# jxx2/MetaFEM.jl

Hardware: AMD Instinct MI355X
Metric: DOF-updates/sec (assembly+CG iter) on 3D hex thermal conduction (higher is better)
Workload: dtype f64; 1 GPU; 3D thermal conduction, linear hex-8, 512x512x512 structured mesh (make_Brick): fused assembly (K + R) + 200 Jacobi-CG iterations per step; n_dof=135005697, nnz=3630961153, parallelism=single GPU

## Files before the change

include/metafem_mi355x_debug.h:

```cpp
#ifndef METAFEM_MI355X_DEBUG_H
#define METAFEM_MI355X_DEBUG_H

#include "metafem_mi355x.h"

#ifdef __cplusplus
extern "C" {
#endif

int64_t mfem_debug_sym_spmv_count(void);
long long mfem_debug_symp_fingerprint_count(void);
long long mfem_debug_symp_coded_count(void);
long long mfem_debug_symp_trim_count(void);
long long mfem_debug_symp_const_count(void);
long long mfem_debug_symp_const_steps(void);
int mfem_debug_spmv_scaled_layout(mfem_context ctx, mfem_csr A, const double* vals, const double* ssym, const double* x, double* y, double alpha, double beta,
                                  const double* dotw, double* partials_out , int32_t cap, int32_t* n_partials , int32_t* form );
int mfem_debug_set(const char* key, int64_t a, int64_t b);

int mfem_debug_lat27_cg_fused(void);
int64_t mfem_debug_lat27_pass1_bytes(mfem_csr A);
long long mfem_debug_lat27_spmv_count(void);
double mfem_debug_lat27_asymmetry(mfem_csr A);
long long mfem_debug_lat8_spmv_count(void);
double mfem_debug_lat8_asymmetry(mfem_csr A);
int mfem_debug_graph_comm_count(void);
long long mfem_debug_graph_launch_count(void);
int64_t mfem_debug_mesh_rows_count(void);
int64_t mfem_debug_mesh_direct_count(void);
int64_t mfem_debug_ws_bytes(mfem_context ctx);
int64_t mfem_debug_mesh_residual_count(void);
int64_t mfem_debug_mesh_operator_count(void);
int64_t mfem_debug_brick_operator_count(void);
int mfem_debug_brick_operator_apply_dot(mfem_context ctx, uint64_t op, const double* x, double* y, double alpha, double beta, const double* dotw,
                                        double* partials, int32_t* n_partials );
int64_t mfem_debug_mesh_ops_count(void);
int64_t mfem_debug_mesh_variants(int32_t reset);
int64_t mfem_debug_op_wave_count(int32_t kernel);
int64_t mfem_debug_sell_periodic_blocks(mfem_csr A);
int64_t mfem_debug_hex27_rows_count(void);
int64_t mfem_debug_hex27_mixed_count(void);
int64_t mfem_debug_hex27_direct_count(void);
int mfem_prof_spmv_enable(mfem_context ctx, int on);
int mfem_prof_spmv_read(mfem_context ctx, double* total_ms , int64_t* launches , int reset);
int mfem_prof_comm_enable(mfem_context ctx, int on);
int mfem_prof_comm_read(mfem_context ctx, double* halo_wait_ms , int64_t* halo_waits , double* allreduce_ms ,
                        int64_t* allreduces , int reset);
int mfem_debug_comm_selftest(mfem_context ctx, int64_t count, int32_t rounds);

unsigned long long mfem_debug_ws_address(mfem_context ctx);
long long mfem_debug_cg_ring_count(void);

int mfem_debug_ws_trial_log(mfem_context ctx, double* out4);

int mfem_debug_fail_host_alloc(int nth);


int mfem_debug_bsell_fields(mfem_csr A);
long long mfem_debug_bsell_spmv_count(void);
int mfem_debug_remainder_info(mfem_csr A, int64_t* rows , int64_t* entries , double* asym_before );
long long mfem_debug_rem_spmv_count(void);
int mfem_debug_csr_tplan(mfem_csr A, int64_t* bytes , double* build_ms );
int mfem_debug_brick_multigrid_transfer(mfem_context ctx, uint64_t mg, int32_t level, int32_t restriction, const double* in, double* out);
double* mfem_debug_brick_multigrid_coords(uint64_t mg, int32_t level, int32_t dim_id);

#ifdef __cplusplus
}
#endif
#endif
```

metafem.jl_amd/_lib.py:

```python
from __future__ import annotations

import ctypes as C
import os

import torch

_HERE = os.path.dirname(os.path.abspath(__file__))
LIB_PATH = os.path.join(_HERE, "libmetafem_mi355x.so")


class MetaFEMError(RuntimeError):
    pass


def _load():
    if not os.path.exists(LIB_PATH):
        raise ImportError(
            f"{LIB_PATH} is missing: build it with `python -c 'import __graft_entry__ as g; g.build()'` "
            "(or `make -C metafem.jl_amd/csrc`).  There is no CPU fallback.")
    return C.CDLL(LIB_PATH, mode=C.RTLD_GLOBAL)


class _Lib:

    def __init__(self, cdll):
        object.__setattr__(self, "_cdll", cdll)

    def __getattr__(self, name):
        if name.startswith("mfem_debug_set_"):
            key = name[len("mfem_debug_set_"):]
            cdll = self._cdll

            def knob(a=0, b=0, _key=key):
                if _key == "recheck_scale":
                    return cdll.mfem_debug_set(b"recheck_scale_ppm", int(round(float(a) * 1e6)), 0)
                return cdll.mfem_debug_set(_key.encode(), int(a), int(b))
            return knob
        return getattr(self._cdll, name)


lib = _Lib(_load())

c_void_p, c_int, c_int32, c_int64, c_double, c_uint64, c_uint32 = (
    C.c_void_p, C.c_int, C.c_int32, C.c_int64, C.c_double, C.c_uint64, C.c_uint32)


class SolveOptions(C.Structure):
    _fields_ = [("method", c_int32), ("precond", c_int32), ("l_or_s", c_int32), ("maxiter", c_int32),
                ("max_pass", c_int32), ("check_every", c_int32), ("converge_tol", c_double), ("seed", c_uint64),
                ("fixed_iterations", c_int32), ("scale_in_place", c_int32), ("left_precond", c_int32),
                ("cg_variant", c_int32)]


class SolveStats(C.Structure):
    _fields_ = [("passes", c_int32), ("iterations", c_int32), ("final_res", c_double), ("initial_res", c_double),
                ("solve_ms", c_double), ("converged", c_int32), ("spmv_count", c_int32)]


class ThermalParams(C.Structure):
    _fields_ = [("k", c_double), ("h", c_double), ("Tenv", c_double), ("robin_faces", c_uint32), ("fixed_faces", c_uint32),
                ("h_penalty", c_double), ("Tw", c_double)]


class ElasticityParams(C.Structure):
    _fields_ = [("lam", c_double), ("mu", c_double), ("tau", c_double), ("penalty_faces", c_uint32),
                ("traction_faces", c_uint32), ("sig", c_double * 6)]


class KvalTerm(C.Structure):
    _fields_ = [("dual_sd", c_int32), ("base_sd", c_int32), ("block", c_int32), ("reserved", c_int32)]


class ResBatchTerm(C.Structure):
    _fields_ = [("dual_sd", c_int32), ("reserved", c_int32), ("cpID_shift", c_int64)]


class VarBatchTerm(C.Structure):
    _fields_ = [("sd", c_int32), ("reserved", c_int32), ("cpID_shift", c_int64), ("x", C.c_void_p)]


class ConstTerm(C.Structure):
    _fields_ = [("dual_sd", c_int32), ("base_sd", c_int32), ("block", c_int32), ("reserved", c_int32), ("coef", c_double)]


MAX_BATCH_TERMS = 48


class MeshDirectStats(C.Structure):
    _fields_ = [(n, c_int64) for n in ("batches", "tasks", "max_batch_doubles", "max_batch_elements", "geometry_evaluations", "device_bytes",
                                       "waves_per_trip", "max_control_point_doubles", "budget_doubles", "waves_per_workgroup", "lds_bytes",
                                       "split_owners", "max_batch_owners")]


class ResSymbol(C.Structure):
    _fields_ = [("word", c_int32), ("reserved", c_int32), ("shift", c_int64), ("x", C.c_void_p)]


class AffineTerm(C.Structure):
    _fields_ = [("dual_pos", c_int32), ("dual_sd", c_int32), ("n_pairs", c_int32), ("reserved", c_int32), ("c0", c_double),
                ("sym", c_int32 * 8), ("normal", c_int32 * 8), ("coef", c_double * 8)]


MAX_RES_SYMBOLS, MAX_RES_TERMS, MAX_RES_PAIRS = 16, 48, 8


class OperatorTerm(C.Structure):
    _fields_ = [("dual_sd", c_int32), ("base_sd", c_int32), ("block", c_int32), ("reserved", c_int32), ("coef", c_double),
                ("normal_coef", c_double * 3)]


MG_MAX_LEVELS = 12


class MultigridOptions(C.Structure):
    _fields_ = [("smoother_degree", c_int32), ("coarse_degree", c_int32), ("smoothing_range", c_double), ("coarse_range", c_double),
                ("eig_steps", c_int32), ("max_levels", c_int32)]


class MultigridInfo(C.Structure):
    _fields_ = [("levels", c_int32), ("sign", c_int32), ("nx", c_int32 * 12), ("ny", c_int32 * 12), ("nz", c_int32 * 12),
                ("lambda_max", c_double * 12), ("products", c_int64 * 12), ("setup_products", c_int64), ("bytes", c_int64), ("cycles", c_int64),
                ("setups", c_int64)]


ALLREDUCE_CB = C.CFUNCTYPE(c_int, c_void_p, C.POINTER(c_double), c_int32)
EXCHANGE_CB = C.CFUNCTYPE(c_int, c_void_p, C.POINTER(c_double), C.POINTER(c_double), C.POINTER(c_double), C.POINTER(c_double), c_int64)


class CommHostOps(C.Structure):
    _fields_ = [("user", c_void_p), ("allreduce_sum", ALLREDUCE_CB), ("neighbour_exchange", EXCHANGE_CB), ("flags", c_uint32),
                ("reserved", c_uint32)]


COMM_HOST_POISON_GHOSTS = 1


class OpLayout(C.Structure):
    _fields_ = [("itg", c_int32), ("itp", c_int32), ("n_sd", c_int32), ("n_host", c_int64), ("index_base", c_int32),
                ("n_colours", c_int32), ("colour_offsets", C.POINTER(c_int64))]


P = c_void_p
SIGNATURES = {
    "mfem_abi_version": (c_int, []),
    "mfem_last_error": (C.c_char_p, []),
    "mfem_context_create": (c_int, [c_int, P, C.POINTER(P)]),
    "mfem_context_set_stream": (c_int, [P, P]),
    "mfem_context_destroy": (c_int, [P]),
    "mfem_context_sync": (c_int, [P]),
    "mfem_csr_create": (c_int, [P, c_int64, c_int64, P, c_int, P, c_int, C.POINTER(P)]),
    "mfem_csr_destroy": (c_int, [P]),
    "mfem_spmv_csr": (c_int, [P, P, P, P, P, c_double, c_double]),
    "mfem_spmv_csr_t": (c_int, [P, P, P, P, P, c_double, c_double]),
    "mfem_axpby": (c_int, [P, c_int64, c_double, P, c_double, P]),
    "mfem_dot": (c_int, [P, c_int64, P, P, C.POINTER(c_double)]),
    "mfem_nrm2": (c_int, [P, c_int64, P, C.POINTER(c_double)]),
    "mfem_rand": (c_int, [P, c_int64, c_uint64, c_uint32, P]),
    "mfem_jacobi_by_diagonal": (c_int, [P, P, P, P]),
    "mfem_jacobi2_by_column": (c_int, [P, P, P, P]),
    "mfem_jacobi_by_row": (c_int, [P, P, P, P]),
    "mfem_mat_div_jacobi": (c_int, [P, P, P, P]),
    "mfem_debug_hex27_direct_count": (c_int64, []),
    "mfem_debug_hex27_mixed_count": (c_int64, []),
    "mfem_debug_hex27_rows_count": (c_int64, []),
    "mfem_debug_mesh_rows_count": (c_int64, []),
    "mfem_debug_mesh_variants": (c_int64, [c_int32]),
    "mfem_debug_op_wave_count": (c_int64, [c_int32]),
    "mfem_debug_bsell_fields": (c_int, [P]),
    "mfem_debug_bsell_spmv_count": (c_int64, []),
    "mfem_debug_sell_periodic_blocks": (c_int64, [P]),
    "mfem_debug_symp_fingerprint_count": (C.c_longlong, []),
    "mfem_debug_symp_coded_count": (C.c_longlong, []),
    "mfem_debug_symp_trim_count": (C.c_longlong, []),
    "mfem_debug_symp_const_count": (C.c_longlong, []),
    "mfem_debug_symp_const_steps": (C.c_longlong, []),
    "mfem_debug_spmv_scaled_layout": (c_int, [P, P, P, P, P, P, c_double, c_double, P, P, c_int32, C.POINTER(c_int32), C.POINTER(c_int32)]),
    "mfem_debug_set": (c_int, [C.c_char_p, c_int64, c_int64]),
    "mfem_debug_graph_comm_count": (c_int, []),
    "mfem_debug_graph_launch_count": (C.c_longlong, []),
    "mfem_debug_cg_ring_count": (C.c_longlong, []),
    "mfem_debug_lat27_cg_fused": (c_int, []),
    "mfem_debug_lat27_pass1_bytes": (c_int64, [P]),
    "mfem_prof_spmv_enable": (c_int, [P, c_int]),
    "mfem_prof_spmv_read": (c_int, [P, C.POINTER(c_double), C.POINTER(c_int64), c_int]),
    "mfem_prof_comm_enable": (c_int, [P, c_int]),
    "mfem_prof_comm_read": (c_int, [P, C.POINTER(c_double), C.POINTER(c_int64), C.POINTER(c_double), C.POINTER(c_int64), c_int]),
    "mfem_solve": (c_int, [P, P, P, P, P, C.POINTER(SolveOptions), C.POINTER(SolveStats)]),
    "mfem_solve_set_shadow": (c_int, [P, P, c_int32]),
    "mfem_brick_create": (c_int, [P, c_int32, c_int32, c_int32, c_double, c_double, c_double, c_int32, c_int32,
                                  C.POINTER(P)]),
    "mfem_brick_destroy": (c_int, [P]),
    "mfem_brick_num_controlpoints": (c_int64, [P]),
    "mfem_brick_num_elements": (c_int64, [P]),
    "mfem_brick_coords": (P, [P, c_int32]),
    "mfem_brick_set_slab": (c_int, [P, c_int32, c_int32]),
    "mfem_brick_pattern": (c_int, [P, P, c_int32, C.POINTER(P)]),
    "mfem_pattern_build": (c_int, [P, c_int32, c_int64, c_int64, P, c_int32, c_int32, C.POINTER(P), P]),
    "mfem_csr_rowptr64": (P, [P]),
    "mfem_csr_colidx": (P, [P]),
    "mfem_csr_nnz": (c_int64, [P]),
    "mfem_csr_n": (c_int64, [P]),
    "mfem_brick_assemble_thermal": (c_int, [P, P, P, C.POINTER(ThermalParams), P]),
    "mfem_brick_residual_thermal": (c_int, [P, P, C.POINTER(ThermalParams), P, P, P]),
    "mfem_brick_assemble_elasticity": (c_int, [P, P, P, C.POINTER(ElasticityParams), P]),
    "mfem_brick_residual_elasticity": (c_int, [P, P, C.POINTER(ElasticityParams), P, P]),
    "mfem_update_basic_elements": (c_int, [P, c_int32, c_int32, c_int32, c_int64, c_int64, P, P, P, P, c_int32, P, P]),
    "mfem_update_basic_boundary": (c_int, [P, c_int32, c_int32, c_int32, c_int32, c_int64, c_int64, P, P, P, P, P, P, P,
                                          c_int32, P, P, P]),
    "mfem_op_var": (c_int, [P, C.POINTER(OpLayout), P, c_int32, c_int64, P, P, P, P, P, c_int64]),
    "mfem_op_kval": (c_int, [P, C.POINTER(OpLayout), P, c_int32, c_int32, P, P, c_int64, P, P, P, c_int64]),
    "mfem_op_res": (c_int, [P, C.POINTER(OpLayout), P, c_int32, P, c_int64, P, P, P, P, c_int64]),
    "mfem_debug_lat27_spmv_count": (c_int64, []),
    "mfem_debug_lat27_asymmetry": (C.c_double, [c_void_p]),
    "mfem_debug_lat8_spmv_count": (c_int64, []),
    "mfem_debug_lat8_asymmetry": (C.c_double, [c_void_p]),
    "mfem_spmv_solver_layout": (c_int, [P, P, P, P, P, c_double, c_double]),
    "mfem_spmv_solver_layout_dot": (c_int, [P, P, P, P, P, c_double, c_double, C.POINTER(c_double)]),
    "mfem_csr_solver_layout": (c_int, [P, P, C.POINTER(c_int32), C.POINTER(c_int32), C.POINTER(c_int64), C.POINTER(c_int64)]),
    "mfem_csr_solver_layout_entries": (c_int, [P, P, C.POINTER(c_int64), C.POINTER(c_int32)]),
    "mfem_csr_solver_layout_bytes": (c_int, [P, P, C.POINTER(c_int64)]),
    "mfem_debug_sym_spmv_count": (c_int64, []),
    "mfem_op_kval_batch": (c_int, [P, C.POINTER(OpLayout), P, c_int32, C.POINTER(KvalTerm), P, P, c_int64, c_int64, P, P, P, c_int64]),
    "mfem_op_res_batch": (c_int, [P, C.POINTER(OpLayout), P, c_int32, C.POINTER(ResBatchTerm), P, P, P, P, P, c_int64]),
    "mfem_op_var_batch": (c_int, [P, C.POINTER(OpLayout), P, c_int32, C.POINTER(VarBatchTerm), P, P, P, P, c_int64]),
    "mfem_mesh_assemble_elements": (c_int, [P, c_int32, c_int32, c_int32, c_int64, c_int64, P, P, P, P, c_int32, c_int32,
                                            C.POINTER(ConstTerm), P, c_int64, P, P, c_int64, c_int32, C.POINTER(c_int64)]),
    "mfem_mesh_assemble_elements_rows": (c_int, [P, c_int32, c_int32, c_int32, c_int64, c_int64, P, P, P, P, c_int32, c_int32,
                                                 C.POINTER(ConstTerm), c_int32, P, P, P, P, P]),
    "mfem_mesh_assemble_elements_rows_set": (c_int, [P, c_int32, c_int32, c_int32, c_int64, c_int64, P, P, P, P, c_int32, c_int32,
                                                 C.POINTER(ConstTerm), c_int32, P, P, P, P, P]),
    "mfem_mesh_direct_plan_create": (c_int, [P, c_int32, c_int64, c_int64, c_int32, P, P, P, P, c_int32, P, C.POINTER(c_uint64)]),
    "mfem_mesh_direct_plan_destroy": (c_int, [c_uint64]),
    "mfem_mesh_direct_plan_stats": (c_int, [c_uint64, C.POINTER(MeshDirectStats)]),
    "mfem_mesh_assemble_elements_direct": (c_int, [P, c_int32, c_int32, c_int32, c_int64, c_int64, P, P, P, P, c_int32, c_int32,
                                                   C.POINTER(ConstTerm), c_int32, P, c_uint64, P, c_int32]),
    "mfem_debug_mesh_direct_count": (c_int64, []),
    "mfem_debug_ws_bytes": (c_int64, [P]),
    "mfem_mesh_row_ranks": (c_int, [P, c_int32, c_int64, c_int64, c_int32, P, P, P, P, c_int32, P]),
    "mfem_mesh_assemble_facets": (c_int, [P, c_int32, c_int32, c_int32, c_int32, c_int64, c_int64, P, P, P, P, P, P, P, c_int32,
                                          c_int32, C.POINTER(ConstTerm), P, c_int64, P, P, c_int64, c_int32, C.POINTER(c_int64)]),
    "mfem_mesh_residual_elements": (c_int, [P, c_int32, c_int32, c_int32, c_int64, c_int64, P, P, P, P, c_int32, c_int32,
                                            C.POINTER(ResSymbol), c_int32, C.POINTER(AffineTerm), P, P, P]),
    "mfem_mesh_residual_facets": (c_int, [P, c_int32, c_int32, c_int32, c_int32, c_int64, c_int64, P, P, P, P, P, P, P, c_int32,
                                          c_int32, C.POINTER(ResSymbol), c_int32, C.POINTER(AffineTerm), P, P, P]),
    "mfem_debug_mesh_residual_count": (c_int64, []),
    "mfem_mesh_operator_create": (c_int, [P, c_int32, c_int32, c_int64, c_int64, c_int32, P, P, c_int32, C.POINTER(c_uint64)]),
    "mfem_mesh_operator_set_elements": (c_int, [c_uint64, c_int32, P, P, P, P, c_int32, C.POINTER(OperatorTerm)]),
    "mfem_mesh_operator_add_facets": (c_int, [c_uint64, c_int32, c_int32, c_int64, P, P, P, P, P, P, P, c_int32, C.POINTER(OperatorTerm),
                                              C.POINTER(c_int32)]),
    "mfem_mesh_operator_set_terms": (c_int, [c_uint64, c_int32, c_int32, C.POINTER(OperatorTerm)]),
    "mfem_mesh_operator_set_variable_terms": (c_int, [c_uint64, c_int32, c_int32, C.POINTER(KvalTerm), P]),
    "mfem_mesh_operator_destroy": (c_int, [c_uint64]),
    "mfem_mesh_operator_apply": (c_int, [P, c_uint64, P, P, c_double, c_double]),
    "mfem_mesh_operator_diagonal": (c_int, [P, c_uint64, P]),
    "mfem_solve_operator": (c_int, [P, c_uint64, P, P, C.POINTER(SolveOptions), C.POINTER(SolveStats)]),
    "mfem_debug_mesh_operator_count": (c_int64, []),
    "mfem_brick_operator_create": (c_int, [P, P, C.POINTER(ThermalParams), C.POINTER(c_uint64)]),
    "mfem_brick_operator_set_params": (c_int, [c_uint64, C.POINTER(ThermalParams)]),
    "mfem_brick_operator_create_elasticity": (c_int, [P, P, C.POINTER(ElasticityParams), C.POINTER(c_uint64)]),
    "mfem_brick_operator_set_elasticity_params": (c_int, [c_uint64, C.POINTER(ElasticityParams)]),
    "mfem_brick_operator_create_hex27": (c_int, [P, P, C.POINTER(ThermalParams), C.POINTER(c_uint64)]),
    "mfem_brick_operator_destroy": (c_int, [c_uint64]),
    "mfem_brick_operator_apply": (c_int, [P, c_uint64, P, P, c_double, c_double]),
    "mfem_brick_operator_diagonal": (c_int, [P, c_uint64, P]),
    "mfem_debug_brick_operator_count": (c_int64, []),
    "mfem_debug_brick_operator_apply_dot": (c_int, [P, c_uint64, P, P, c_double, c_double, P, P, C.POINTER(c_int32)]),
    "mfem_brick_multigrid_create": (c_int, [P, c_uint64, C.POINTER(MultigridOptions), C.POINTER(c_uint64)]),
    "mfem_brick_multigrid_create_elasticity": (c_int, [P, c_uint64, C.POINTER(MultigridOptions), C.POINTER(c_uint64)]),
    "mfem_brick_multigrid_setup": (c_int, [P, c_uint64]),
    "mfem_brick_multigrid_apply": (c_int, [P, c_uint64, P, P]),
    "mfem_brick_multigrid_info": (c_int, [c_uint64, C.POINTER(MultigridInfo)]),
    "mfem_brick_multigrid_destroy": (c_int, [c_uint64]),
    "mfem_debug_brick_multigrid_transfer": (c_int, [P, c_uint64, c_int32, c_int32, P, P]),
    "mfem_debug_brick_multigrid_coords": (P, [c_uint64, c_int32, c_int32]),
    "mfem_mesh_var_elements": (c_int, [P, c_int32, c_int32, c_int32, c_int64, c_int64, P, P, P, P, c_int32, c_int32,
                                       C.POINTER(VarBatchTerm), P, P, c_int64]),
    "mfem_mesh_var_facets": (c_int, [P, c_int32, c_int32, c_int32, c_int32, c_int64, c_int64, P, P, P, P, P, P, P, c_int32,
                                     c_int32, C.POINTER(VarBatchTerm), P, P, P, c_int64]),
    "mfem_mesh_res_elements": (c_int, [P, c_int32, c_int32, c_int32, c_int64, c_int64, P, P, P, P, c_int32, c_int32,
                                       C.POINTER(ResBatchTerm), P, P, P, P, P]),
    "mfem_mesh_res_facets": (c_int, [P, c_int32, c_int32, c_int32, c_int32, c_int64, c_int64, P, P, P, P, P, P, P, c_int32,
                                     c_int32, C.POINTER(ResBatchTerm), P, P, P, P, P]),
    "mfem_mesh_kval_elements": (c_int, [P, c_int32, c_int32, c_int32, c_int64, c_int64, P, P, P, P, c_int32, c_int32,
                                        C.POINTER(KvalTerm), P, P, c_int64, P, P, c_int64, c_int32, C.POINTER(c_int64)]),
    "mfem_mesh_kval_elements_rows": (c_int, [P, c_int32, c_int32, c_int32, c_int64, c_int64, P, P, P, P, c_int32, c_int32,
                                             C.POINTER(KvalTerm), P, P, c_int32, P, P, P, P, P]),
    "mfem_mesh_kval_facets": (c_int, [P, c_int32, c_int32, c_int32, c_int32, c_int64, c_int64, P, P, P, P, P, P, P, c_int32,
                                      c_int32, C.POINTER(KvalTerm), P, P, c_int64, P, P, c_int64, c_int32, C.POINTER(c_int64)]),
    "mfem_debug_mesh_ops_count": (c_int64, []),
    "mfem_comm_unique_id": (c_int, [P]),
    "mfem_comm_create": (c_int, [P, c_int32, c_int32, P, C.POINTER(P)]),
    "mfem_comm_destroy": (c_int, [P]),
    "mfem_context_set_comm": (c_int, [P, P, c_int64, c_int64, c_int32]),
    "mfem_allreduce_sum": (c_int, [P, P, c_int32]),
    "mfem_halo_exchange": (c_int, [P, P]),
    "mfem_halo_reduce": (c_int, [P, P]),
    "mfem_comm_create_host": (c_int, [P, c_int32, c_int32, C.POINTER(CommHostOps), C.POINTER(P)]),
    "mfem_csr_ncols": (c_int64, [P]),
    "mfem_csr_replan": (c_int, [P, P]),
    "mfem_csr_spmv_bytes": (c_int, [P, P, C.POINTER(c_int64), C.POINTER(c_int64)]),
    "mfem_debug_comm_selftest": (c_int, [P, c_int64, c_int32]),
    "mfem_debug_ws_address": (C.c_ulonglong, [P]),
    "mfem_debug_fail_host_alloc": (c_int, [c_int]),
    "mfem_debug_ws_trial_log": (c_int, [P, C.POINTER(C.c_double)]),
    "mfem_debug_remainder_info": (c_int, [P, C.POINTER(c_int64), C.POINTER(c_int64), C.POINTER(C.c_double)]),
    "mfem_debug_rem_spmv_count": (C.c_longlong, []),
    "mfem_debug_csr_tplan": (c_int, [P, C.POINTER(c_int64), C.POINTER(C.c_double)]),
}

for _name, (_res, _args) in SIGNATURES.items():
    _fn = getattr(lib, _name)
    _fn.restype = _res
    _fn.argtypes = _args


def check(rc: int) -> None:
    if rc != 0:
        raise MetaFEMError(f"libmetafem_mi355x rc={rc}: {lib.mfem_last_error().decode()}")
```

metafem.jl_amd/csrc/api.hip:

```cpp
#include <stdarg.h>
#include <atomic>

#include <exception>
#include <mutex>
#include <new>
#include <set>

#include "common.h"
#include <string>

static std::mutex g_ctx_mutex;
static std::set<mfem_context_s*> g_live_contexts;
bool mfem_context_alive(mfem_context_s* ctx) {
  std::lock_guard<std::mutex> lk(g_ctx_mutex);
  return g_live_contexts.count(ctx) != 0;
}

static thread_local char g_err[1024] = "";

void mfem_set_error(const char* fmt, ...) {
  va_list ap;
  va_start(ap, fmt);
  vsnprintf(g_err, sizeof(g_err), fmt, ap);
  va_end(ap);
}

int mfem_api_exception(const char* entry) noexcept {
  try {
    throw;
  } catch (const std::bad_alloc&) {
    mfem_set_error("%s: host memory exhausted (std::bad_alloc)", entry);
    return MFEM_ERR_ALLOC;
  } catch (const std::exception& e) {
    mfem_set_error("%s: internal error: %s", entry, e.what());
    return MFEM_ERR_INTERNAL;
  } catch (...) {
    mfem_set_error("%s: internal error (unknown C++ exception)", entry);
    return MFEM_ERR_INTERNAL;
  }
}

static std::atomic<int> g_fail_host_alloc{0};
extern "C" int mfem_debug_fail_host_alloc(int nth) try {
  g_fail_host_alloc.store(nth > 0 ? nth : 0);
  return MFEM_OK;
} MFEM_API_CATCH("mfem_debug_fail_host_alloc")
void mfem_host_alloc_probe() {
  int v = g_fail_host_alloc.load();
  while (v > 0) {
    if (g_fail_host_alloc.compare_exchange_weak(v, v - 1)) {
      if (v == 1) throw std::bad_alloc();
      return;
    }
  }
}

std::atomic<int> mfem_debug_epoch{0};

extern "C" int mfem_abi_version(void) { return MFEM_ABI_VERSION; }
extern "C" const char* mfem_last_error(void) { return g_err; }

int mfem_ws_release(void* raw);
static int context_allocate(mfem_context_s* c) {
  MFEM_CHECK_HIP(hipMalloc(&c->d_partials, sizeof(double) * MFEM_MAX_PARTIALS * 8));
  MFEM_CHECK_HIP(hipMalloc(&c->d_scalars, sizeof(double) * MFEM_NSCALARS));
  MFEM_CHECK_HIP(hipHostMalloc(&c->h_scalars, sizeof(double) * MFEM_NSCALARS));
  MFEM_CHECK_HIP(hipMalloc(&c->d_flags, sizeof(int32_t) * MFEM_NFLAGS));
  MFEM_CHECK_HIP(hipHostMalloc(&c->h_flags, sizeof(int32_t) * MFEM_NFLAGS));
  MFEM_CHECK_HIP(hipMemsetAsync(c->d_scalars, 0, sizeof(double) * MFEM_NSCALARS, c->stream));
  MFEM_CHECK_HIP(hipMemsetAsync(c->d_flags, 0, sizeof(int32_t) * MFEM_NFLAGS, c->stream));
  MFEM_CHECK_HIP(hipEventCreate(&c->ev0));
  MFEM_CHECK_HIP(hipEventCreate(&c->ev1));
  return MFEM_OK;
}

static void context_release(mfem_context_s* ctx) {
  if (ctx->d_partials) hipFree(ctx->d_partials);
  if (ctx->d_scalars) hipFree(ctx->d_scalars);
  if (ctx->h_scalars) hipHostFree(ctx->h_scalars);
  if (ctx->d_flags) hipFree(ctx->d_flags);
  if (ctx->h_flags) hipHostFree(ctx->h_flags);
  (void)mfem_ws_release(ctx->ws_raw);
  (void)mfem_ws_release(ctx->ws_alt_raw);
  if (ctx->prof_ev) {
    for (int i = 0; i < 2 * MFEM_PROF_PAIRS; ++i)
      if (ctx->prof_ev[i]) hipEventDestroy(ctx->prof_ev[i]);
    delete[] ctx->prof_ev;
  }
  if (ctx->ev0) hipEventDestroy(ctx->ev0);
  if (ctx->ev1) hipEventDestroy(ctx->ev1);
  for (int i = 0; i < MFEM_GRAPH_SLOTS; ++i)
    if (ctx->graph_exec[i]) hipGraphExecDestroy(ctx->graph_exec[i]);
  if (ctx->graph_ev) hipEventDestroy(ctx->graph_ev);
  if (ctx->graph_stream) hipStreamDestroy(ctx->graph_stream);
}

extern "C" int mfem_context_create(int device, void* stream, mfem_context* out) try {
  MFEM_REQUIRE(out != nullptr, "out is null");
  int ndev = 0;
  MFEM_CHECK_HIP(hipGetDeviceCount(&ndev));
  MFEM_REQUIRE(device >= 0 && device < ndev, "no such HIP device");
  MFEM_CHECK_HIP(hipSetDevice(device));
  hipDeviceProp_t prop;
  MFEM_CHECK_HIP(hipGetDeviceProperties(&prop, device));
  if (strncmp(prop.gcnArchName, "gfx950", 6) != 0) {
    mfem_set_error("libmetafem_mi355x is built for gfx950 only, device %d is %s", device, prop.gcnArchName);
    return MFEM_ERR_UNSUPPORTED;
  }
  mfem_host_alloc_probe();
  mfem_context_s* c = new mfem_context_s();
  memset(c, 0, sizeof(*c));
  c->device = device;
  c->stream = (hipStream_t)stream;
  c->num_cus = prop.multiProcessorCount;
  int rc = context_allocate(c);
  if (rc != MFEM_OK) {
    context_release(c);
    delete c;
    return rc;
  }
  {
    std::lock_guard<std::mutex> lk(g_ctx_mutex);
    g_live_contexts.insert(c);
  }
  *out = c;
  return MFEM_OK;
} MFEM_API_CATCH("mfem_context_create")

extern "C" int mfem_context_set_stream(mfem_context ctx, void* stream) try {
  MFEM_REQUIRE(ctx != nullptr, "ctx is null");
  ctx->stream = (hipStream_t)stream;
  return MFEM_OK;
} MFEM_API_CATCH("mfem_context_set_stream")

extern "C" int mfem_context_sync(mfem_context ctx) try {
  MFEM_REQUIRE(ctx != nullptr, "ctx is null");
  MFEM_CHECK_HIP(hipStreamSynchronize(ctx->stream));
  return MFEM_OK;
} MFEM_API_CATCH("mfem_context_sync")

extern "C" int mfem_context_destroy(mfem_context ctx) try {
  if (!ctx) return MFEM_OK;
  {
    std::lock_guard<std::mutex> lk(g_ctx_mutex);
    g_live_contexts.erase(ctx);
  }
  hipStreamSynchronize(ctx->stream);
  context_release(ctx);
  delete ctx;
  return MFEM_OK;
} MFEM_API_CATCH("mfem_context_destroy")

int mfem_prof_flush(mfem_context_s* ctx) {
  if (ctx->prof_used == 0) return MFEM_OK;
  MFEM_CHECK_HIP(hipEventSynchronize(ctx->prof_ev[2 * ctx->prof_used - 1]));
  for (int k = 0; k < ctx->prof_used; ++k) {
    float ms = 0.f;
    MFEM_CHECK_HIP(hipEventElapsedTime(&ms, ctx->prof_ev[2 * k], ctx->prof_ev[2 * k + 1]));
    ctx->prof_ms += ms;
  }
  ctx->prof_count += ctx->prof_used;
  ctx->prof_used = 0;
  return MFEM_OK;
}

extern "C" int mfem_prof_spmv_enable(mfem_context ctx, int on) try {
  MFEM_REQUIRE(ctx, "null ctx");
  if (on && !ctx->prof_ev) {
    ctx->prof_ev = new hipEvent_t[2 * MFEM_PROF_PAIRS]();
    for (int i = 0; i < 2 * MFEM_PROF_PAIRS; ++i) MFEM_CHECK_HIP(hipEventCreate(&ctx->prof_ev[i]));
  }
  if (!on) {
    int rc = mfem_prof_flush(ctx);
    if (rc) return rc;
  }
  ctx->prof_on = on ? 1 : 0;
  return MFEM_OK;
} MFEM_API_CATCH("mfem_prof_spmv_enable")

extern "C" int mfem_prof_spmv_read(mfem_context ctx, double* total_ms, int64_t* launches, int reset) try {
  MFEM_REQUIRE(ctx && total_ms && launches, "null argument");
  int rc = mfem_prof_flush(ctx);
  if (rc) return rc;
  *total_ms = ctx->prof_ms;
  *launches = ctx->prof_count;
  if (reset) {
    ctx->prof_ms = 0.0;
    ctx->prof_count = 0;
  }
  return MFEM_OK;
} MFEM_API_CATCH("mfem_prof_spmv_read")

uint64_t mfem_next_csr_serial() {
  static std::atomic<uint64_t> next{1};
  return next.fetch_add(1);
}

void mfem_graphs_invalidate(mfem_context_s* ctx) {
  for (int i = 0; i < MFEM_GRAPH_SLOTS; ++i)
    if (ctx->graph_exec[i]) {
      hipGraphExecDestroy(ctx->graph_exec[i]);
      ctx->graph_exec[i] = nullptr;
      ctx->graph_key[i] = 0;
    }
}

static std::atomic<size_t> g_ws_align{0}, g_ws_offset{0};
extern "C" int mfem_debug_set_ws_placement(long long align, long long offset) try {
  g_ws_align = align > 0 ? (size_t)align : 0;
  g_ws_offset = offset > 0 ? (size_t)offset : 0;
  return MFEM_OK;
} MFEM_API_CATCH("mfem_debug_set_ws_placement")
static int ws_alloc(mfem_context_s* ctx, void** raw, size_t bytes) {
  (void)ctx;
  *raw = nullptr;
  MFEM_CHECK_HIP(hipMalloc(raw, bytes));
  return MFEM_OK;
}
static int ws_free(void* raw) {
  if (raw) MFEM_CHECK_HIP(hipFree(raw));
  return MFEM_OK;
}
int mfem_ws_release(void* raw) { return ws_free(raw); }
extern "C" int64_t mfem_debug_ws_bytes(mfem_context ctx) { return ctx ? (int64_t)ctx->ws_bytes : 0; }
extern "C" unsigned long long mfem_debug_ws_address(mfem_context ctx) { return ctx ? (unsigned long long)(uintptr_t)ctx->ws : 0ull; }
#include <chrono>
static double now_ms() { return std::chrono::duration<double, std::milli>(std::chrono::steady_clock::now().time_since_epoch()).count(); }
int mfem_ws_next_candidate(mfem_context_s* ctx) {
  const bool verbose = getenv("MFEM_WS_TRIAL_VERBOSE") != nullptr;
  double t0 = now_ms();
  MFEM_CHECK_HIP(hipStreamSynchronize(ctx->stream));
  if (verbose) fprintf(stderr, "ws trial: sync %.1f ms\n", now_ms() - t0);
  const size_t need = ctx->ws_bytes + g_ws_align + g_ws_offset;
  if (ctx->ws_alt_raw) {
    t0 = now_ms();
    {
      int rcf = ws_free(ctx->ws_raw);
      if (rcf) return rcf;
    }
    if (verbose) fprintf(stderr, "ws trial: free %.1f ms\n", now_ms() - t0);
    ctx->ws = ctx->ws_raw = nullptr;
  }
  size_t freeb = 0, totalb = 0;
  void* raw = nullptr;
  bool ok = hipMemGetInfo(&freeb, &totalb) == hipSuccess && freeb >= need + ((size_t)4 << 30);
  t0 = now_ms();
  if (ok && ws_alloc(ctx, &raw, need) != MFEM_OK) ok = false;
  if (verbose) fprintf(stderr, "ws trial: alloc %.1f ms\n", now_ms() - t0);
  if (!ok) {
    (void)hipGetLastError();
    if (!ctx->ws_raw) {
      ctx->ws = ctx->ws_alt;
      ctx->ws_raw = ctx->ws_alt_raw;
      ctx->ws_alt = ctx->ws_alt_raw = nullptr;
    }
    return MFEM_OK;
  }
  if (ctx->ws_raw) {
    ctx->ws_alt = ctx->ws;
    ctx->ws_alt_raw = ctx->ws_raw;
  }
  ctx->ws_raw = raw;
  uintptr_t p = (uintptr_t)raw;
  if (g_ws_align) p = (p + g_ws_align - 1) / g_ws_align * g_ws_align;
  ctx->ws = (void*)(p + g_ws_offset);
  ctx->ws_try += 1;
  return MFEM_OK;
}
int mfem_ws_decide(mfem_context_s* ctx, bool keep_current) {
  MFEM_CHECK_HIP(hipStreamSynchronize(ctx->stream));
  if (ctx->ws_alt_raw) {
    if (keep_current) {
      int rcf = ws_free(ctx->ws_alt_raw);
      if (rcf) return rcf;
    } else {
      int rcf = ws_free(ctx->ws_raw);
      if (rcf) return rcf;
      ctx->ws = ctx->ws_alt;
      ctx->ws_raw = ctx->ws_alt_raw;
    }
  }
  ctx->ws_alt = ctx->ws_alt_raw = nullptr;
  ctx->ws_try = 99;
  return MFEM_OK;
}
int mfem_ws_reserve(mfem_context_s* ctx, size_t bytes) {
  if (bytes <= ctx->ws_bytes) return MFEM_OK;
  MFEM_CHECK_HIP(hipStreamSynchronize(ctx->stream));
  int rcf = ws_free(ctx->ws_raw);
  if (!rcf) rcf = ws_free(ctx->ws_alt_raw);
  ctx->ws = ctx->ws_raw = ctx->ws_alt = ctx->ws_alt_raw = nullptr;
  ctx->ws_try = 0;
  ctx->ws_bytes = 0;
  if (rcf) return rcf;
  rcf = ws_alloc(ctx, &ctx->ws_raw, bytes + g_ws_align + g_ws_offset);
  if (rcf) return rcf;
  uintptr_t p = (uintptr_t)ctx->ws_raw;
  if (g_ws_align) p = (p + g_ws_align - 1) / g_ws_align * g_ws_align;
  ctx->ws = (void*)(p + g_ws_offset);
  ctx->ws_bytes = bytes;
  return MFEM_OK;
}

extern "C" {
int mfem_debug_set_spmv(int, int);
int mfem_debug_set_ell(int);
int mfem_debug_set_sell(int);
int mfem_debug_set_lat27(int);
int mfem_debug_set_lat8(int);
int mfem_debug_set_layout_min_rows(int64_t, int64_t);
int mfem_debug_set_graphs(int, int64_t);
int mfem_debug_set_idrs(int);
int mfem_debug_set_bicgstabl(int);
int mfem_debug_set_gmres(int);
int mfem_debug_set_vec_grid(int);
int mfem_debug_set_halo_overlap(int);
int mfem_debug_set_hex27(int);
int mfem_debug_set_elasticity(int);
int mfem_debug_set_hex8_thermal(int);
int mfem_debug_set_ws_placement(long long, long long);
int mfem_debug_set_ws_trial(int);
int mfem_debug_set_cg_streaming(int);
int mfem_debug_set_cg_ring(int);
int mfem_debug_set_cg_single_max_rows(int64_t);
int mfem_debug_set_csr_strips(int, int64_t);
int mfem_debug_set_remainder(int);
int mfem_debug_set_recheck_scale(double);
int mfem_debug_set_bsell(int);
}
extern int g_mesh_gather_rows, g_mesh_abl, g_mesh_stage_min_itp, g_mesh_term_matrix;
extern int g_op_wave_forms, g_op_wave_min_itp;
extern int64_t g_mesh_direct_budget;
extern "C" int mfem_debug_set(const char* key, int64_t a, int64_t b) try {
  MFEM_REQUIRE(key, "null key");
  const std::string k(key);
  if (k == "spmv") return mfem_debug_set_spmv((int)a, (int)b);
  if (k == "ell") return mfem_debug_set_ell((int)a);
  if (k == "sell") return mfem_debug_set_sell((int)a);
  if (k == "lat27") return mfem_debug_set_lat27((int)a);
  if (k == "lat8") return mfem_debug_set_lat8((int)a);
  if (k == "layout_min_rows") return mfem_debug_set_layout_min_rows(a, b);
  if (k == "graphs") return mfem_debug_set_graphs((int)a, b);
  if (k == "idrs") return mfem_debug_set_idrs((int)a);
  if (k == "bicgstabl") return mfem_debug_set_bicgstabl((int)a);
  if (k == "gmres") return mfem_debug_set_gmres((int)a);
  if (k == "vec_grid") return mfem_debug_set_vec_grid((int)a);
  if (k == "halo_overlap") return mfem_debug_set_halo_overlap((int)a);
  if (k == "hex27") return mfem_debug_set_hex27((int)a);
  if (k == "elasticity") return mfem_debug_set_elasticity((int)a);
  if (k == "hex8_thermal") return mfem_debug_set_hex8_thermal((int)a);
  if (k == "ws_placement") return mfem_debug_set_ws_placement((long long)a, (long long)b);
  if (k == "ws_trial") return mfem_debug_set_ws_trial((int)a);
  if (k == "cg_streaming") return mfem_debug_set_cg_streaming((int)a);
  if (k == "cg_ring") return mfem_debug_set_cg_ring((int)a);
  if (k == "cg_single_max_rows") return mfem_debug_set_cg_single_max_rows(a);
  if (k == "csr_strips") return mfem_debug_set_csr_strips((int)a, b);
  if (k == "remainder") return mfem_debug_set_remainder((int)a);
  if (k == "mesh_gather_rows") { g_mesh_gather_rows = (int)a; return MFEM_OK; }
  if (k == "bsell") return mfem_debug_set_bsell((int)a);
  if (k == "op_wave_forms") { g_op_wave_forms = (int)a; g_op_wave_min_itp = b > 0 ? (int)b : 10; return MFEM_OK; }
  if (k == "mesh_stage_min_itp") { g_mesh_stage_min_itp = a > 0 ? (int)a : 16; return MFEM_OK; }
  if (k == "mesh_term_matrix") { g_mesh_term_matrix = (int)a; return MFEM_OK; }
  if (k == "mesh_direct_budget") { g_mesh_direct_budget = a > 0 ? a : 0; return MFEM_OK; }
  if (k == "mesh_abl") { g_mesh_abl = (int)a; return MFEM_OK; }
  if (k == "recheck_scale_ppm") return mfem_debug_set_recheck_scale((double)a * 1e-6);
  mfem_set_error("mfem_debug_set: unknown key '%s'", key);
  return MFEM_ERR_INVALID;
} MFEM_API_CATCH("mfem_debug_set")
```

metafem.jl_amd/csrc/common.h:

```cpp
#pragma once
#include <hip/hip_runtime.h>
#include <atomic>
#include <mutex>
#include <unordered_map>
#include <stdint.h>
#include <stdio.h>
#include <string.h>

#if defined(__HIP_DEVICE_COMPILE__) && !defined(__gfx950__)
#error "metafem_mi355x is written for gfx950 (MI355X) only: counted s_waitcnt vmcnt(k) pipelines assume loads and stores share one in-order counter, global_load_lds_dwordx4 and v_mfma_f64 are used directly -- build with --offload-arch=gfx950"
#endif
#include "../../include/metafem_mi355x.h"
#include "../../include/metafem_mi355x_debug.h"
#include "csr_decide.h"
#include "sell_decide.h"
#include "lat_decide.h"

#define MFEM_WAVE 64
#define MFEM_BLOCK 256
#define MFEM_MAX_PARTIALS 4096
static_assert(LAT_MAX_GATHER_GRID == MFEM_MAX_PARTIALS, "a workgroup of the tiles' gather pass writes one partial sum");
#define MFEM_NFLAGS 80
#define MFEM_NSCALARS 4096

void mfem_set_error(const char* fmt, ...);

int mfem_api_exception(const char* entry) noexcept;
#define MFEM_API_CATCH(entry) catch (...) { return mfem_api_exception(entry); }
void mfem_host_alloc_probe();

#define MFEM_CHECK_HIP(expr)                                                                  \
  do {                                                                                        \
    hipError_t _e = (expr);                                                                   \
    if (_e != hipSuccess) {                                                                   \
      mfem_set_error("%s:%d: %s -> %s", __FILE__, __LINE__, #expr, hipGetErrorString(_e));    \
      return MFEM_ERR_HIP;                                                                    \
    }                                                                                         \
  } while (0)

#define MFEM_REQUIRE(cond, msg)                                      \
  do {                                                               \
    if (!(cond)) {                                                   \
      mfem_set_error("%s:%d: %s (%s)", __FILE__, __LINE__, msg, #cond); \
      return MFEM_ERR_INVALID;                                       \
    }                                                                \
  } while (0)

#define MFEM_CHECK_LAUNCH() MFEM_CHECK_HIP(hipGetLastError())

template <typename T> struct __attribute__((visibility("hidden"))) DevBuf {
  T* p = nullptr;
  DevBuf() = default;
  DevBuf(DevBuf&& o) noexcept : p(o.release()) {}
  DevBuf& operator=(DevBuf&& o) noexcept { if (this != &o) { reset(); p = o.release(); } return *this; }
  DevBuf(const DevBuf&) = delete;
  DevBuf& operator=(const DevBuf&) = delete;
  ~DevBuf() { reset(); }
  hipError_t alloc(size_t count) { reset(); return hipMalloc((void**)&p, sizeof(T) * count); }
  void reset() { if (p) (void)hipFree(p); p = nullptr; }
  T* release() { T* q = p; p = nullptr; return q; }
  operator T*() const { return p; }
};

struct mfem_comm_s;

#define MFEM_MAX_ZONES 8
struct SpmvPart {
  int part;
  int nz;
  int64_t lo[MFEM_MAX_ZONES], hi[MFEM_MAX_ZONES];
};
__host__ __device__ __forceinline__ bool spmv_part_skip(const SpmvPart& P, int64_t r0, int64_t r1) {
  if (P.part == 0) return false;
  bool bnd = false;
  for (int z = 0; z < P.nz; ++z) bnd = bnd || (r0 < P.hi[z] && r1 > P.lo[z]);
  return P.part == 1 ? bnd : !bnd;
}


#define MFEM_GRAPH_SLOTS 4
struct mfem_context_s {
  int device;
  hipStream_t stream;
  int num_cus;
  double* d_partials;
  double* d_scalars;
  double* h_scalars;
  int32_t* d_flags;
  int32_t* h_flags;
  void* ws;
  void* ws_raw;
  size_t ws_bytes;
  int ws_try;
  void* ws_alt;
  void* ws_alt_raw;
  float ws_try_ms;
  float ws_log[4];
  const double* shadow;
  int32_t shadow_count;
  mfem_comm_s* comm;
  int64_t halo_plane_len;
  int32_t halo_fields;
  hipEvent_t ev0, ev1;
  int prof_on;
  int prof_used;
  hipEvent_t* prof_ev;
  double prof_ms;
  int64_t prof_count;
  hipGraphExec_t graph_exec[MFEM_GRAPH_SLOTS];
  uint64_t graph_key[MFEM_GRAPH_SLOTS];
  int graph_next;
  hipStream_t graph_stream;
  hipEvent_t graph_ev;
  int graph_active;
  int force_csr;
  int probe_active;
};
#define MFEM_PROF_PAIRS 1024
int mfem_prof_flush(mfem_context_s* ctx);

struct mfem_operator_head;
struct mfem_csr_s {
  mfem_context_s* ctx;
  uint64_t serial;
  int64_t n, nnz;
  const void* rowptr;
  int rowptr_bits;
  const int32_t* colidx;
  int index_base;
  int32_t max_row_nnz;
  CsrPlan plan;
  int nb_F, nb_checked;
  int64_t rb_ntiles;
  int64_t rb_elided;
  int32_t* rb_rows;
  uint8_t* cw_elide;
  int32_t lat_m1, lat_m2, lat_fields;
  int32_t lat_m0, lat_plo, lat_gw;
  int32_t lat_inferred;
  uint16_t* diag_off;
  void* owned_rowptr;
  void* owned_colidx;
  int64_t x_offset;
  int64_t ncols;
  int ell_state, ell_K;
  int64_t ell_npad;
  int32_t* ell_cols;
  const double* ell_src;
  double* ell_vals;
  int dia_state, dia_classes;
  void* dia_dev;
  int32_t* dia_flags;
  int32_t dia_regular_blocks;
  int dia_triples;
  int sym_state;
  int64_t sym_c0, sym_c1;
  int sym_cls;
  int sym_S;
  int64_t sym_mx, sym_myz;
  int ell_bound_mode;
  int dia_kernel;
  int symp_state;
  int symp_m1, symp_m2;
  int64_t symp_PL;
  int symp_p0, symp_p1;
  int symp_NS, symp_NPk;
  int symp_B;
  int symp_trim;
  int symp_DC;
  int symp_dneg;
  int symp_CS;
  int symp_cs_last;
  int64_t symp_flagged, symp_flagged_last;
  double symp_cst[27];
  int symp_ccode;
  int symp_dc_last;
  double* symp_vals;
  SellLayout sell;
  LatTiles lat27, lat8;
  int lat_refused;
  int rem_active;
  int64_t rem_nrows, rem_nent, rem_cap_rows, rem_cap_ent;
  int32_t* rem_rows;
  int64_t* rem_ptr;
  int32_t* rem_len;
  int32_t* rem_col;
  double* rem_val;
  unsigned long long* rem_cnt;
  void* rem_sort_tmp;
  size_t rem_sort_bytes;
  double rem_asym_before;
  int64_t rem_last_rows, rem_last_ent;
  struct mfem_tplan_s* tplan;
  struct mfem_operator_head* op;
  double* op_scratch;
  const double* op_dsc;
  uint64_t op_epoch;
};
struct mfem_tplan_s {
  mfem_csr_s* AT;
  void* perm;
  int perm_bits;
  double* vals;
  int64_t bytes;
  double build_ms;
};
static inline CsrShape mfem_csr_shape(const mfem_csr_s* A) { return {A->n, A->nnz, A->max_row_nnz}; }
template <typename F> static inline auto mfem_by_rowptr(const mfem_csr_s* A, F&& f) { return A->rowptr_bits == 64 ? f(int64_t{}) : f(int32_t{}); }
int mfem_tplan_get(mfem_context_s* ctx, mfem_csr_s* A, mfem_tplan_s** out);
void mfem_tplan_free(mfem_csr_s* A);
int mfem_tplan_gather(mfem_context_s* ctx, const mfem_tplan_s* P, const double* src, double* valsT, const double* d1, const double* d2);
bool mfem_rem_enabled();
bool mfem_rem_diag();
void mfem_rem_clear(mfem_csr_s* A);
void mfem_rem_free(mfem_csr_s* A);
int mfem_rem_build(mfem_context_s* ctx, mfem_csr_s* A, const double* vals, int n_fields, const double* y1, const double* y2, const double* scale,
                   double gate, bool* built);
int mfem_rem_apply(mfem_context_s* ctx, mfem_csr_s* A, const double* x, const double* dsc, double* y, double alpha, const double* dotw,
                   double* partials, int* n_partials, const int32_t* done_flag);
int64_t mfem_rem_design_bytes(const mfem_csr_s* A);
int mfem_spmv_lat8_launch(mfem_context_s* ctx, mfem_csr_s* A, const double* vals, const double* x, double* y, double alpha, double beta,
                          const double* dotw, double* partials, int* n_partials, const int32_t* done_flag, int part);
int64_t mfem_lat8_design_bytes(const mfem_csr_s* A);
int64_t mfem_lat8_entries(const mfem_csr_s* A);
int mfem_lattice_hint_from_row0(mfem_context_s* ctx, mfem_csr_s* A);
static inline LatShape mfem_lat_shape(const mfem_csr_s* A, int64_t min_rows) {
  return {A->n, A->ncols, A->max_row_nnz, A->lat_m0, A->lat_m1, A->lat_m2, A->lat_fields, A->lat_plo, A->lat_gw, min_rows};
}
static inline void mfem_lat_unbind(mfem_csr_s* A, LatTiles& T) {
  if (T.vals) A->rem_active = 0;
  T.vals = T.dump = nullptr;
  T.src = T.dsc = nullptr;
}
int mfem_sym_probe(mfem_context_s* ctx, mfem_csr_s* A, LatTiles* T, const double* vals, double* scratch, double amax, double* asym, int rem_fields);
int mfem_spmv_lat27_launch(mfem_context_s* ctx, mfem_csr_s* A, const double* vals, const double* x, double* y, double alpha,
                           double beta, const double* dotw, double* partials, int* n_partials, const int32_t* done_flag, int part);
int64_t mfem_lat27_design_bytes(const mfem_csr_s* A);
int64_t mfem_lat27_entries(const mfem_csr_s* A);
int mfem_node_block_fields(mfem_context_s* ctx, mfem_csr_s* A);
int mfem_spmv_sell_launch(mfem_context_s* ctx, mfem_csr_s* A, const double* vals, const double* x, double* y, double alpha,
                          double beta, const double* dotw, double* partials, int* n_partials, const int32_t* done_flag, int part);
int mfem_ell_diag(mfem_context_s* ctx, mfem_csr_s* A, double* d);
int mfem_spmv_ell_launch(mfem_context_s* ctx, mfem_csr_s* A, const double* vals, const double* x, double* y, double alpha,
                         double beta, const double* dotw, double* partials, int* n_partials, const int32_t* done_flag,
                         const SpmvPart& part);
struct SpmvArgs {
  const double* x; double* y; double alpha, beta; const double* dotw; double* partials; int* n_partials; const int32_t* done_flag; const SpmvPart& part;
};
__attribute__((visibility("hidden"))) int mfem_spmv_csr_launch(mfem_context_s* ctx, mfem_csr_s* A, const double* vals, const double* x, double* y, double alpha,
                                                             double beta, const double* dotw, double* partials, int* n_partials, const int32_t* done_flag,
                                                             const SpmvPart& part);
__attribute__((visibility("hidden"))) CsrKnobs mfem_csr_knobs();

enum mfem_layout : int32_t { MFEM_LAYOUT_CSR = 0, MFEM_LAYOUT_ELL = 1, MFEM_LAYOUT_DIA = 2, MFEM_LAYOUT_SELL = 3, MFEM_LAYOUT_LAT27 = 4, MFEM_LAYOUT_LAT8 = 5,
                             MFEM_LAYOUT_OPERATOR = 6  };
struct mfem_layout_plan_s {
  mfem_layout tile, rows;
  size_t tile_bytes, rows_bytes;
};
int mfem_layout_plan(mfem_context_s* ctx, mfem_csr_s* A, bool is_cg, bool allow_tiles, mfem_layout_plan_s* P);
int mfem_layout_bind(mfem_context_s* ctx, mfem_csr_s* A, mfem_layout mode, const double* vals, double* buf, const double* dsc, const double* ssym,
                     double* scratch, bool allow_rem);
mfem_layout mfem_layout_bound(const mfem_csr_s* A, const double* vals);
void mfem_layout_unbind(mfem_csr_s* A);
void mfem_layout_drop(mfem_csr_s* A);

int mfem_ws_reserve(mfem_context_s* ctx, size_t bytes);
int mfem_ws_next_candidate(mfem_context_s* ctx);
int mfem_ws_decide(mfem_context_s* ctx, bool keep_current);
uint64_t mfem_next_csr_serial();
bool mfem_context_alive(mfem_context_s* ctx);
void mfem_graphs_invalidate(mfem_context_s* ctx);
extern std::atomic<int> mfem_debug_epoch;

__device__ __forceinline__ double wave_reduce_sum(double v) {
#pragma unroll
  for (int off = 32; off > 0; off >>= 1) v += __shfl_down(v, off, MFEM_WAVE);
  return v;
}

__device__ __forceinline__ void mfem_lds_barrier() { asm volatile("s_waitcnt lgkmcnt(0)\n\ts_barrier" ::: "memory"); }

__device__ __forceinline__ bool mfem_xcd_tile(int tcount, int& tsub) {
  const int chunk = (tcount + 7) >> 3;
  tsub = (int)(blockIdx.x & 7) * chunk + (int)(blockIdx.x >> 3);
  return !((int)(blockIdx.x >> 3) >= chunk || tsub >= tcount);
}

__device__ __forceinline__ double block_reduce_sum(double v, double* smem ) {
  v = wave_reduce_sum(v);
  const int lane = threadIdx.x & 63, w = threadIdx.x >> 6;
  __syncthreads();
  if (lane == 0) smem[w] = v;
  __syncthreads();
  double r = 0.0;
  if (threadIdx.x == 0) {
    const int nw = (blockDim.x + 63) >> 6;
    for (int i = 0; i < nw; ++i) r += smem[i];
  }
  __syncthreads();
  return r;
}

static inline int mfem_resident_per_cu(const void* kernel, int block_threads, size_t dyn_lds, int fallback) {
  static std::mutex mu;
  static std::unordered_map<const void*, int> cache;
  std::lock_guard<std::mutex> lk(mu);
  auto it = cache.find(kernel);
  if (it != cache.end()) return it->second;
  int occ = 0;
  const hipError_t e = hipOccupancyMaxActiveBlocksPerMultiprocessor(&occ, kernel, block_threads, dyn_lds);
  const int v = (e == hipSuccess && occ >= 1) ? occ : fallback;
  cache[kernel] = v;
  return v;
}
static inline int mfem_grid_for(int64_t work_items, int per_block, int cap) {
  int64_t g = (work_items + per_block - 1) / per_block;
  if (g < 1) g = 1;
  if (g > cap) g = cap;
  return (int)g;
}
```

metafem.jl_amd/csrc/spmv_ell.h:

```cpp
#pragma once
#include <vector>

#include "layouts.h"
#include "spmv_symp.h"
#include "symp_trim_decide.h"
#include "symp_const_decide.h"

#define ELL_B 128
__host__ __device__ __forceinline__ int64_t ell_base(int64_t r, int K) { return (r >> 7) * ((int64_t)K * ELL_B) + (r & (ELL_B - 1)); }

typedef double e_d2 __attribute__((ext_vector_type(2)));
typedef int e_i2 __attribute__((ext_vector_type(2)));
typedef double u_d2 __attribute__((ext_vector_type(2), aligned(8)));

#define DIA_MAXD 96
#define DIA_MAXC 4
struct DiaOffsets {
  int ncls;
  int D[DIA_MAXC];
  int32_t off[DIA_MAXC][DIA_MAXD];
};

struct SympGeom {
  int64_t PL, nx;
  int m1, m2, p0, p1, NS, NPk;
  int nseg;
  int B, NR;
  int DC;
  long long unit;
  int ms1, ms2;
  int rim_pp;
  int64_t rim_rows, rim_units;
};
struct SympConst {
  double v[27];
  int32_t code, valid;
};
#define SPC_COUNT_AT 20
#define SPC_REF_AT 22
static_assert(SPC_REF_AT % 2 == 0 && SPC_REF_AT * 4 + sizeof(SympConst) <= MFEM_NFLAGS * 4, "the reference row must fit the context's flags");
struct SympTail {
  int on, K;
  int rim;
  int64_t n, npad, lo, hi;
  const DiaOffsets* Op;
  const int32_t* flags;
  const int32_t* cols;
  const double* ell;
};

#if defined(DV_ABL) && DV_ABL == 1
#define DIA_ST(p, v) do { if ((v) == 1.2345e300) __builtin_nontemporal_store((v), (p)); } while (0)
#elif defined(DV_ABL) && DV_ABL == 3
#define DIA_ST(p, v) (*(p) = (v))
#else
#define DIA_ST(p, v) __builtin_nontemporal_store((v), (p))
#endif
#define SYM_LD(p) __builtin_nontemporal_load(p)

template <int RPT, int U, bool TRIPLES>
__device__ __forceinline__ void dia_rows(int64_t r, int64_t n, int64_t npad, int K, const DiaOffsets& O,
                                         const int32_t* __restrict__ flags, const int32_t* __restrict__ cols,
                                         const double* __restrict__ vals, const double* __restrict__ x, double* __restrict__ y,
                                         double alpha, double beta, const double* __restrict__ dotw, int xcd, double& dot_acc,
                                         int64_t skip_lo = 0, int64_t skip_hi = 0) {
  constexpr int H = RPT / 2;
  const double* v = vals + ell_base(r, K);
  e_d2 acc[H];
  double xself0 = 0.0, xself1 = 0.0;
  bool have_self = false;
#pragma unroll
  for (int h = 0; h < H; ++h) acc[h] = (e_d2){0.0, 0.0};
  const int64_t blk = r / (64 * RPT) * (RPT / 2);
  const int cls = __builtin_amdgcn_readfirstlane(flags[blk]) - 1;
  bool interior = cls >= 0;
  if (RPT == 4) interior = interior && ((blk + 1) * 128 < npad) && flags[blk + 1] == cls + 1;
  const int32_t* off = O.off[cls < 0 ? 0 : cls];
  const int D = O.D[cls < 0 ? 0 : cls];
  if (interior && TRIPLES && RPT == 2) {
    for (int s = 0; s < D; s += 3) {
      const e_d2 va = __builtin_nontemporal_load(reinterpret_cast<const e_d2*>(v + s * ELL_B));
      const e_d2 vb = __builtin_nontemporal_load(reinterpret_cast<const e_d2*>(v + (s + 1) * ELL_B));
      const e_d2 vc = __builtin_nontemporal_load(reinterpret_cast<const e_d2*>(v + (s + 2) * ELL_B));
      const u_d2* xp = reinterpret_cast<const u_d2*>(x + r + off[s]);
      const u_d2 xa = xp[0], xb = xp[1];
      acc[0].x += va.x != 0.0 ? va.x * xa.x : 0.0;
      acc[0].y += va.y != 0.0 ? va.y * xa.y : 0.0;
      acc[0].x += vb.x != 0.0 ? vb.x * xa.y : 0.0;
      acc[0].y += vb.y != 0.0 ? vb.y * xb.x : 0.0;
      acc[0].x += vc.x != 0.0 ? vc.x * xb.x : 0.0;
      acc[0].y += vc.y != 0.0 ? vc.y * xb.y : 0.0;
      if (off[s + 1] == 0) {
        xself0 = xa.y;
        xself1 = xb.x;
        have_self = true;
      }
    }
  } else if (interior) {
    int s = 0;
    for (; s + U <= D; s += U) {
      e_d2 vv[U][H];
      u_d2 xx[U][H];
#pragma unroll
      for (int u = 0; u < U; ++u)
#pragma unroll
        for (int h = 0; h < H; ++h) {
          vv[u][h] = __builtin_nontemporal_load(reinterpret_cast<const e_d2*>(v + (s + u) * ELL_B) + h);
          xx[u][h] = *(reinterpret_cast<const u_d2*>(x + r + off[s + u]) + h);
        }
#pragma unroll
      for (int u = 0; u < U; ++u)
#pragma unroll
        for (int h = 0; h < H; ++h) {
          acc[h].x += vv[u][h].x != 0.0 ? vv[u][h].x * xx[u][h].x : 0.0;
          acc[h].y += vv[u][h].y != 0.0 ? vv[u][h].y * xx[u][h].y : 0.0;
        }
    }
    for (; s < D; ++s)
#pragma unroll
      for (int h = 0; h < H; ++h) {
        const e_d2 vv = __builtin_nontemporal_load(reinterpret_cast<const e_d2*>(v + s * ELL_B) + h);
        const u_d2 xx = *(reinterpret_cast<const u_d2*>(x + r + off[s]) + h);
        acc[h].x += vv.x != 0.0 ? vv.x * xx.x : 0.0;
        acc[h].y += vv.y != 0.0 ? vv.y * xx.y : 0.0;
      }
  } else {
    const int32_t* c = cols + ell_base(r, K);
    for (int s = 0; s < K; ++s)
#pragma unroll
      for (int h = 0; h < H; ++h) {
        if (r + 2 * h >= npad) continue;
        const e_d2 vv = __builtin_nontemporal_load(reinterpret_cast<const e_d2*>(v + s * ELL_B) + h);
        const e_i2 cc = __builtin_nontemporal_load(reinterpret_cast<const e_i2*>(c + s * ELL_B) + h);
        acc[h].x += vv.x * x[cc.x];
        acc[h].y += vv.y * x[cc.y];
      }
  }
#pragma unroll
  for (int h = 0; h < H; ++h) {
    const int64_t rr = r + 2 * h;
    if (rr >= n) break;
    double y0 = alpha * acc[h].x, y1 = alpha * acc[h].y;
    const bool one = rr < skip_lo || rr >= skip_hi;
    const bool two = rr + 1 < n && (rr + 1 < skip_lo || rr + 1 >= skip_hi);
    if (beta != 0.0) {
      if (one) y0 += beta * y[rr];
      if (two) y1 += beta * y[rr + 1];
    }
    if (one) y[rr] = y0;
    if (two) y[rr + 1] = y1;
    if (dotw) {
      if (RPT == 2 && have_self && dotw == x) {
        if (one) dot_acc += y0 * xself0;
        if (two) dot_acc += y1 * xself1;
      } else {
        if (one) dot_acc += y0 * dotw[rr];
        if (two) dot_acc += y1 * dotw[rr + 1];
      }
    }
  }
}

struct EllKnobs {
  std::atomic<int> enable{1};
  std::atomic<int> dia{1};
  std::atomic<int> symp_trim{0};
  std::atomic<int> symp_const{0};
  std::atomic<int> grid_mult{6};
  std::atomic<int> shared_x{1};
  std::atomic<int> xcd{0};
  std::atomic<int> symp_coded{1};
  std::atomic<int> sym{1};
  std::atomic<int> symp{1};
  std::atomic<int> symp_bands{0};
  std::atomic<int> symp_tail{1};
  std::atomic<int> symp_direct{1};
  std::atomic<int> dia_pipe{1};
  std::atomic<int> dia_fast{1};
  std::atomic<int> symp_fingerprint{1};
};
extern EllKnobs g_ell;
extern std::atomic<int64_t> g_layout_min_rows_dia, g_layout_min_rows_cols;

enum DiaKernel : int { DIA_NONE = 0, DIA_ROWS, DIA_ROWS_TRIPLES, DIA_SYM27, DIA_SYMP };
DiaKernel mfem_dia_kernel_wanted(const mfem_csr_s* A, DiaKernel refused = DIA_NONE, bool* direct = nullptr);
int mfem_dia_plan(mfem_context_s* ctx, mfem_csr_s* A);
int mfem_dia_copy(mfem_context_s* ctx, mfem_csr_s* A, const double* vals, double* buf, const double* dsc, const double* ssym, const SympGeom& G,
                  double* pvals, double* rim, bool want_fp, bool* fp_made, unsigned char* sflags = nullptr, bool* flags_made = nullptr);
int mfem_dia_launch(mfem_context_s* ctx, mfem_csr_s* A, bool triples, int cap, const SpmvArgs& a);
int mfem_dia_launch_outside(mfem_context_s* ctx, mfem_csr_s* A, const SpmvArgs& a, double* partials, int64_t lo, int64_t hi, int* ngrid);
void mfem_sym_plan(mfem_csr_s* A, const int32_t* off, int lc, int64_t m2, int64_t PL, int64_t run_lo, int64_t run_hi);
bool mfem_sym_wanted(const mfem_csr_s* A, DiaKernel k);
SympGeom mfem_symp_geom(const mfem_context_s* ctx, const mfem_csr_s* A);
int64_t mfem_symp_steps(const mfem_csr_s* A, int B = 0, int trim = -1);
int mfem_symp_bands_wanted(const mfem_csr_s* A);
int mfem_symp_bands(const mfem_csr_s* A);
int mfem_symp_trim_wanted(const mfem_csr_s* A);
int mfem_symp_trim(const mfem_csr_s* A);
int64_t mfem_symp_copy_doubles(const mfem_csr_s* A, int B, int trim);
int64_t mfem_symp_swept_rows(const mfem_csr_s* A);
int mfem_symp_coded_wanted(DiaKernel k, bool fast, const double* ssym);
int mfem_symp_coded(const mfem_csr_s* A);
bool mfem_dia_fill_fast(const mfem_csr_s* A, const double* dsc, bool direct);
int64_t mfem_sym_entries(const mfem_context_s* ctx, const mfem_csr_s* A, DiaKernel k);
int mfem_sym_verdict(mfem_context_s* ctx, mfem_csr_s* A, DiaKernel k, const double* buf, double* pvals, const SympGeom& G, bool direct, bool fp_made, bool* ok,
                     bool* dc_refused, int* dneg, bool flags_made = false, SympConst* cst = nullptr, int64_t* flagged = nullptr);
unsigned char* mfem_symp_flags_of(double* pvals, const SympGeom& G);
int mfem_sym_launch(mfem_context_s* ctx, mfem_csr_s* A, DiaKernel k, const SpmvArgs& a);
```

metafem.jl_amd/csrc/spmv_ell.hip:

```cpp
#include "blas1.h"
#include "spmv_ell.h"

std::atomic<int64_t> g_layout_min_rows_dia{262144};
std::atomic<int64_t> g_layout_min_rows_cols{1000000};
#define LAT27_MIN_ROWS 180000
std::atomic<int64_t> g_layout_min_rows_lat27{LAT27_MIN_ROWS};
extern "C" int mfem_debug_set_layout_min_rows(int64_t diagonal_slots, int64_t explicit_columns) try {
  ++mfem_debug_epoch;
  g_layout_min_rows_dia = diagonal_slots;
  g_layout_min_rows_cols = explicit_columns;
  g_layout_min_rows_lat27 = explicit_columns < LAT27_MIN_ROWS ? explicit_columns : LAT27_MIN_ROWS;
  return MFEM_OK;
} MFEM_API_CATCH("mfem_debug_set_layout_min_rows")

EllKnobs g_ell;
extern "C" int mfem_debug_set_ell(int enable) try {
  ++mfem_debug_epoch;
  g_ell.enable = enable & 1;
  g_ell.dia = (enable & 2) ? 0 : 1;
  g_ell.symp_trim = (enable & 4) ? 2 : (enable & 8) ? 1 : 0;
  g_ell.symp_const = (enable & 16) ? 2 : (enable & 32) ? 1 : 0;
  if ((enable >> 8) & 255) g_ell.grid_mult = (enable >> 8) & 255;
  g_ell.shared_x = ((enable >> 16) & 15) == 8 ? 0 : 1;
  g_ell.xcd = (enable >> 20) & 1;
  g_ell.symp_coded = ((enable >> 21) & 1) ? 0 : 1;
  g_ell.sym = ((enable >> 22) & 1) ? 0 : 1;
  g_ell.symp = ((enable >> 23) & 1) ? 0 : 1;
  g_ell.symp_bands = ((enable >> 24) & 1) ? 1 : ((enable >> 25) & 1) ? 2 : 0;
  g_ell.symp_tail = ((enable >> 26) & 1) ? 0 : 1;
  g_ell.symp_direct = ((enable >> 27) & 1) ? 0 : 1;
  g_ell.dia_pipe = ((enable >> 28) & 1) ? 0 : 1;
  g_ell.dia_fast = ((enable >> 29) & 1) ? 0 : 1;
  g_ell.symp_fingerprint = ((enable >> 30) & 1) ? 0 : 1;
  return MFEM_OK;
} MFEM_API_CATCH("mfem_debug_set_ell")

template <typename RP>
__global__ __launch_bounds__(MFEM_BLOCK) void k_ell_cols(int64_t n, int64_t npad, int K, const RP* __restrict__ rowptr,
                                                           const int32_t* __restrict__ col, int base, int32_t* __restrict__ out) {
  const int64_t stride = (int64_t)gridDim.x * blockDim.x;
  for (int64_t r = blockIdx.x * (int64_t)blockDim.x + threadIdx.x; r < npad; r += stride) {
    int64_t lo = 0;
    int len = 0;
    if (r < n) {
      lo = (int64_t)rowptr[r] - base;
      len = (int)((int64_t)rowptr[r + 1] - base - lo);
    }
    const int32_t self = (int32_t)(r < n ? r : 0);
    for (int s = 0; s < K; ++s) out[ell_base(r, K) + s * ELL_B] = s < len ? col[lo + s] - base : self;
  }
}

template <typename RP>
__global__ __launch_bounds__(MFEM_BLOCK) void k_ell_vals_lds(int64_t n, int64_t npad, int K, const RP* __restrict__ rowptr,
                                                               const double* __restrict__ vals, int base, double* __restrict__ out,
                                                               const int32_t* __restrict__ col, const double* __restrict__ dsc) {
  extern __shared__ double lds[];
  const int lane = threadIdx.x & 63, w = threadIdx.x >> 6, nw = blockDim.x >> 6;
  double* T = lds + (size_t)w * 64 * K;
  const int64_t ntiles = npad >> 6;
  for (int64_t tile = (int64_t)blockIdx.x * nw + w; tile < ntiles; tile += (int64_t)gridDim.x * nw) {
    const int64_t r0 = tile << 6, r = r0 + lane;
    const int64_t rend = (r0 + 64 < n) ? r0 + 64 : n;
    int64_t lo = 0;
    int len = 0;
    if (r < n) {
      lo = (int64_t)rowptr[r] - base;
      len = (int)((int64_t)rowptr[r + 1] - base - lo);
    }
    const int64_t s0 = r0 < n ? (int64_t)rowptr[r0] - base : 0;
    const int cnt = r0 < n ? (int)((int64_t)rowptr[rend] - base - s0) : 0;
    constexpr int NB = 28;
    for (int i0 = lane; i0 < cnt; i0 += 64 * NB) {
      double tv[NB];
#pragma unroll
      for (int u = 0; u < NB; ++u) {
        const int i = i0 + 64 * u;
        tv[u] = i < cnt ? vals[s0 + i] : 0.0;
        if (dsc && i < cnt) tv[u] /= dsc[col[s0 + i] - base];
      }
#pragma unroll
      for (int u = 0; u < NB; ++u) {
        const int i = i0 + 64 * u;
        if (i < cnt) T[i] = tv[u];
      }
    }
    __builtin_amdgcn_wave_barrier();
    __builtin_amdgcn_s_waitcnt(0xC07F);
    const int off = (int)(lo - s0);
    for (int s = 0; s < K; ++s) out[ell_base(r, K) + s * ELL_B] = s < len ? T[off + s] : 0.0;
    __builtin_amdgcn_wave_barrier();
  }
}

template <int RPT, int U>
__global__ __launch_bounds__(MFEM_BLOCK) void k_spmv_ell(int64_t n, int64_t npad, int K, const int32_t* __restrict__ cols,
                                                           const double* __restrict__ vals, const double* __restrict__ x,
                                                           double* __restrict__ y, double alpha, double beta,
                                                           const double* __restrict__ dotw, double* __restrict__ partials,
                                                           const int32_t* __restrict__ done_flag, SpmvPart part) {
  __shared__ double red[4];
  if (done_flag && done_flag[0]) return;
  double dot_acc = 0.0;
  const int64_t stride = (int64_t)gridDim.x * blockDim.x * RPT;
  for (int64_t r = (blockIdx.x * (int64_t)blockDim.x + threadIdx.x) * RPT; r < n; r += stride) {
    if (spmv_part_skip(part, r, r + RPT)) continue;
    const double* v = vals + ell_base(r, K);
    const int32_t* c = cols + ell_base(r, K);
    if (RPT == 1) {
      double acc = 0.0;
      int s = 0;
      for (; s + U <= K; s += U) {
        double vv[U];
        int32_t cc[U];
#pragma unroll
        for (int u = 0; u < U; ++u) {
          vv[u] = __builtin_nontemporal_load(v + (s + u) * ELL_B);
          cc[u] = __builtin_nontemporal_load(c + (s + u) * ELL_B);
        }
#pragma unroll
        for (int u = 0; u < U; ++u) acc += vv[u] * x[cc[u]];
      }
      for (; s < K; ++s) acc += __builtin_nontemporal_load(v + s * ELL_B) * x[__builtin_nontemporal_load(c + s * ELL_B)];
      double yv = alpha * acc;
      if (beta != 0.0) yv += beta * y[r];
      y[r] = yv;
      if (dotw) dot_acc += yv * dotw[r];
    } else {
      e_d2 acc = {0.0, 0.0};
      int s = 0;
      for (; s + U <= K; s += U) {
        e_d2 vv[U];
        e_i2 cc[U];
#pragma unroll
        for (int u = 0; u < U; ++u) {
          vv[u] = __builtin_nontemporal_load(reinterpret_cast<const e_d2*>(v + (s + u) * ELL_B));
          cc[u] = __builtin_nontemporal_load(reinterpret_cast<const e_i2*>(c + (s + u) * ELL_B));
        }
#pragma unroll
        for (int u = 0; u < U; ++u) {
          acc.x += vv[u].x * x[cc[u].x];
          acc.y += vv[u].y * x[cc[u].y];
        }
      }
      for (; s < K; ++s) {
        const e_d2 v1 = __builtin_nontemporal_load(reinterpret_cast<const e_d2*>(v + s * ELL_B));
        const e_i2 c1 = __builtin_nontemporal_load(reinterpret_cast<const e_i2*>(c + s * ELL_B));
        acc.x += v1.x * x[c1.x];
        acc.y += v1.y * x[c1.y];
      }
      double y0 = alpha * acc.x, y1 = alpha * acc.y;
      const bool two = r + 1 < n;
      if (beta != 0.0) {
        y0 += beta * y[r];
        if (two) y1 += beta * y[r + 1];
      }
      y[r] = y0;
      if (two) y[r + 1] = y1;
      if (dotw) {
        dot_acc += y0 * dotw[r];
        if (two) dot_acc += y1 * dotw[r + 1];
      }
    }
  }
  if (partials) {
    const double b = block_reduce_sum(dot_acc, red);
    if (threadIdx.x == 0) partials[blockIdx.x] = b;
  }
}

__global__ __launch_bounds__(MFEM_BLOCK) void k_ell_diag(int64_t n, int K, const DiaOffsets* __restrict__ Op,
                                                           const int32_t* __restrict__ flags, const int32_t* __restrict__ cols,
                                                           const double* __restrict__ vals, double* __restrict__ d) {
  const int64_t stride = (int64_t)gridDim.x * blockDim.x;
  for (int64_t r = blockIdx.x * (int64_t)blockDim.x + threadIdx.x; r < n; r += stride) {
    const int64_t b = ell_base(r, K);
    const int cls = flags ? flags[r >> 7] - 1 : -1;
    double out = 1.0;
    if (cls >= 0) {
      const int D = Op->D[cls];
      for (int s = 0; s < D; ++s)
        if (Op->off[cls][s] == 0) {
          const double v = vals[b + s * ELL_B];
          if (v != 0.0) out = fabs(v);
          break;
        }
    } else {
      for (int s = 0; s < K; ++s)
        if (cols[b + s * ELL_B] == (int32_t)r) {
          const double v = vals[b + s * ELL_B];
          if (v != 0.0) out = fabs(v);
          break;
        }
    }
    d[r] = out;
  }
}

static int ell_plan_columns(mfem_context_s* ctx, mfem_csr_s* A) {
  A->ell_state = -1;
  const int K = A->max_row_nnz;
  if (A->n < 1 || K < 1 || K > 128) return MFEM_OK;
  const int64_t npad = (A->n + ELL_B - 1) & ~(int64_t)(ELL_B - 1);
  if ((double)K * (double)npad > 1.10 * (double)A->nnz + 64.0 * K) return MFEM_OK;
  MFEM_CHECK_HIP(hipMalloc(&A->ell_cols, sizeof(int32_t) * (size_t)K * (size_t)npad));
  const int grid = mfem_grid_for(npad, MFEM_BLOCK, ctx->num_cus * 16);
  mfem_by_rowptr(A, [&](auto t) {
    hipLaunchKernelGGL(k_ell_cols<decltype(t)>, dim3(grid), dim3(MFEM_BLOCK), 0, ctx->stream, A->n, npad, K, (const decltype(t)*)A->rowptr, A->colidx,
                       A->index_base, A->ell_cols);
  });
  MFEM_CHECK_LAUNCH();
  A->ell_K = K;
  A->ell_npad = npad;
  A->ell_state = 1;
  return MFEM_OK;
}
int mfem_ell_plan(mfem_context_s* ctx, mfem_csr_s* A) {
  if (A->ell_state != 0) return MFEM_OK;
  if (A->n < g_layout_min_rows_dia && A->n < g_layout_min_rows_cols) return MFEM_OK;
  struct Undo {
    mfem_csr_s* A;
    ~Undo() {
      if (!A) return;
      mfem_ell_free(A);
      A->sym_state = A->symp_state = 0;
    }
  } undo{A};
  int rc = ell_plan_columns(ctx, A);
  if (!rc && A->ell_state == 1) rc = mfem_dia_plan(ctx, A);
  if (!rc) undo.A = nullptr;
  return rc;
}

bool mfem_dia_layout_planned(const mfem_csr_s* A) { return A->ell_state == 1 && g_ell.enable && A->dia_state == 1 && g_ell.dia; }
DiaKernel mfem_dia_kernel_wanted(const mfem_csr_s* A, DiaKernel refused, bool* direct) {
  DiaKernel k = DIA_ROWS;
  if (A->dia_triples && g_ell.shared_x) {
    k = DIA_ROWS_TRIPLES;
    if (refused != DIA_SYM27 && mfem_sym_wanted(A, DIA_SYM27)) k = DIA_SYM27;
    if (refused == DIA_NONE && mfem_sym_wanted(A, DIA_SYMP)) k = DIA_SYMP;
  }
  if (direct) *direct = k == DIA_SYMP && g_ell.symp_direct;
  return k;
}
#define SYMP_BANDS2_MIN_ROWS 100000000
int mfem_symp_bands_wanted(const mfem_csr_s* A) {
  if (g_ell.symp_bands) return g_ell.symp_bands;
  return A->symp_state == 1 && (int64_t)(A->symp_p1 - A->symp_p0) * A->symp_PL >= SYMP_BANDS2_MIN_ROWS ? 2 : 1;
}
int mfem_symp_bands(const mfem_csr_s* A) { return A->symp_B ? A->symp_B : mfem_symp_bands_wanted(A); }
#define SYMP_TRIM_MIN_ROWS 16000000
int mfem_symp_trim_wanted(const mfem_csr_s* A) {
  if (g_ell.symp_trim) return g_ell.symp_trim == 1 ? 1 : 0;
  return A->symp_state == 1 && (int64_t)(A->symp_p1 - A->symp_p0) * A->symp_PL >= SYMP_TRIM_MIN_ROWS ? 1 : 0;
}
int mfem_symp_trim(const mfem_csr_s* A) { return A->symp_B ? A->symp_trim : mfem_symp_trim_wanted(A); }
static std::atomic<long long> g_symp_trim_binds{0};
extern "C" long long mfem_debug_symp_trim_count(void) { return g_symp_trim_binds; }
int mfem_symp_coded_wanted(DiaKernel k, bool fast, const double* ssym) { return k == DIA_SYMP && fast && ssym && g_ell.symp_coded ? 1 : 0; }
int mfem_symp_coded(const mfem_csr_s* A) { return A->symp_vals ? A->symp_DC : A->symp_dc_last; }
static std::atomic<long long> g_symp_coded_binds{0};
extern "C" long long mfem_debug_symp_coded_count(void) { return g_symp_coded_binds; }
static std::atomic<long long> g_symp_const_binds{0}, g_symp_const_steps{0};
extern "C" long long mfem_debug_symp_const_count(void) { return g_symp_const_binds; }
extern "C" long long mfem_debug_symp_const_steps(void) { return g_symp_const_steps; }
size_t mfem_ell_vals_bytes(const mfem_csr_s* A) {
  if (A->ell_state != 1 || !g_ell.enable) return 0;
  const bool dia = mfem_dia_layout_planned(A);
  if (A->n < (dia ? g_layout_min_rows_dia : g_layout_min_rows_cols)) return 0;
  size_t bytes = sizeof(double) * (size_t)A->ell_K * (size_t)A->ell_npad;
  if (dia && mfem_dia_kernel_wanted(A) == DIA_SYMP) {
    size_t pm = 0;
    for (int B = 1; B <= SP_BMAX; ++B)
      for (int trim = 0; trim <= 1; ++trim) pm = std::max(pm, sizeof(double) * (size_t)mfem_symp_copy_doubles(A, B, trim));
    bytes += pm;
  }
  return bytes;
}
static int dia_bind(mfem_context_s* ctx, mfem_csr_s* A, const double* vals, double* buf, const double* dsc, const double* ssym) {
  bool direct = false, fp_made = false, flags_made = false;
  SympConst cst{};
  int64_t flagged = 0;
  DiaKernel k = mfem_dia_kernel_wanted(A, DIA_NONE, &direct);
  A->symp_trim = mfem_symp_trim_wanted(A);
  A->symp_B = mfem_symp_bands_wanted(A);
  A->symp_DC = mfem_symp_coded_wanted(k, mfem_dia_fill_fast(A, dsc, direct), ssym);
  A->symp_dneg = 0;
  double* pvals = buf + (size_t)A->ell_K * (size_t)A->ell_npad;
  SympGeom G = k == DIA_SYMP ? mfem_symp_geom(ctx, A) : SympGeom{};
  auto rim_of = [&](const SympGeom& g) -> double* { return k == DIA_SYMP && g.rim_units > 0 ? pvals + (int64_t)g.NR * g.NPk * (g.p1 - g.p0) * sp_step(g.B, g.DC) : nullptr; };
  auto flags_of = [&](const SympGeom& g) -> unsigned char* { return k == DIA_SYMP && direct && g_ell.symp_const != 2 ? mfem_symp_flags_of(pvals, g) : nullptr; };
  int rc = mfem_dia_copy(ctx, A, vals, buf, dsc, ssym, G, direct ? pvals : nullptr, rim_of(G), g_ell.symp_fingerprint != 0, &fp_made, flags_of(G), &flags_made);
  while (!rc && (k == DIA_SYMP || k == DIA_SYM27)) {
    bool ok = false, dc_refused = false;
    rc = mfem_sym_verdict(ctx, A, k, buf, pvals, G, direct, fp_made, &ok, &dc_refused, &A->symp_dneg, flags_made, &cst, &flagged);
    if (rc) break;
    if (dc_refused) {
      A->symp_DC = 0;
      G = mfem_symp_geom(ctx, A);
      rc = mfem_dia_copy(ctx, A, vals, buf, dsc, ssym, G, pvals, rim_of(G), g_ell.symp_fingerprint != 0, &fp_made, flags_of(G), &flags_made);
      continue;
    }
    if (ok) break;
    if (k == DIA_SYMP && direct) rc = mfem_dia_copy(ctx, A, vals, buf, dsc, ssym, SympGeom{}, nullptr, nullptr, false, &fp_made);
    k = mfem_dia_kernel_wanted(A, k);
  }
  if (rc) return rc;
  A->ell_vals = buf;
  A->ell_src = vals;
  A->ell_bound_mode = 2;
  A->dia_kernel = k;
  A->symp_vals = k == DIA_SYMP ? pvals : nullptr;
  if (k != DIA_SYMP) A->symp_B = A->symp_DC = A->symp_trim = 0;
  if (!A->symp_DC) A->symp_dneg = 0;
  A->symp_CS = 0;
  A->symp_flagged = 0;
  if (k == DIA_SYMP) {
    const int64_t steps = mfem_symp_steps(A);
    if (!flags_made) flagged = 0;
    bool mirror = fp_made || flagged == 0;
    for (int sl = 0; sl < 13 && mirror && flagged > 0; ++sl) mirror = memcmp(&cst.v[sl], &cst.v[26 - sl], sizeof(double)) == 0;
    A->symp_CS = spc_form(flags_made && mirror, flags_made && cst.valid != 0, flagged, steps, g_ell.symp_const == 2, g_ell.symp_const == 1);
    A->symp_flagged = flagged;
    memcpy(A->symp_cst, cst.v, sizeof(A->symp_cst));
    A->symp_ccode = cst.code;
    A->symp_cs_last = A->symp_CS;
    A->symp_flagged_last = flagged;
    g_symp_const_steps = flagged;
    if (A->symp_CS) ++g_symp_const_binds;
    A->symp_dc_last = A->symp_DC;
    if (A->symp_DC) ++g_symp_coded_binds;
    if (G.rim_units > 0) ++g_symp_trim_binds;
  }
  return MFEM_OK;
}

int mfem_ell_bind(mfem_context_s* ctx, mfem_csr_s* A, const double* vals, double* buf, const double* dsc, const double* ssym) {
  mfem_ell_unbind(A);
  if (A->ell_state != 1 || !g_ell.enable || !buf) return MFEM_OK;
  if (mfem_dia_layout_planned(A)) return dia_bind(ctx, A, vals, buf, dsc, ssym);
  int waves = 4;
  while (waves > 1 && sizeof(double) * 64 * (size_t)A->ell_K * waves > 64 * 1024) waves >>= 1;
  const size_t lds = sizeof(double) * 64 * (size_t)A->ell_K * waves;
  const int64_t ntiles = A->ell_npad >> 6;
  int grid = (int)((ntiles + waves - 1) / waves);
  if (grid > ctx->num_cus * 16) grid = ctx->num_cus * 16;
  mfem_by_rowptr(A, [&](auto t) {
    hipLaunchKernelGGL(k_ell_vals_lds<decltype(t)>, dim3(grid), dim3(64 * waves), lds, ctx->stream, A->n, A->ell_npad, A->ell_K,
                       (const decltype(t)*)A->rowptr, vals, A->index_base, buf, A->colidx, dsc);
  });
  MFEM_CHECK_LAUNCH();
  A->ell_vals = buf;
  A->ell_src = vals;
  A->ell_bound_mode = 1;
  return MFEM_OK;
}
void mfem_ell_unbind(mfem_csr_s* A) {
  A->ell_bound_mode = A->dia_kernel = DIA_NONE;
  A->ell_vals = A->symp_vals = nullptr;
  A->ell_src = nullptr;
  A->symp_B = A->symp_DC = A->symp_dneg = A->symp_trim = A->symp_CS = 0;
  A->symp_flagged = 0;
}
void mfem_ell_free(mfem_csr_s* A) {
  if (A->ell_cols) hipFree(A->ell_cols);
  if (A->dia_flags) hipFree(A->dia_flags);
  if (A->dia_dev) hipFree(A->dia_dev);
  A->ell_cols = nullptr;
  A->dia_flags = nullptr;
  A->dia_dev = nullptr;
  A->ell_state = A->dia_state = 0;
}
int mfem_ell_diag(mfem_context_s* ctx, mfem_csr_s* A, double* d) {
  if (!A->ell_vals) return MFEM_ERR_INVALID;
  const int grid = mfem_grid_for(A->n, MFEM_BLOCK, ctx->num_cus * 16);
  hipLaunchKernelGGL(k_ell_diag, dim3(grid), dim3(MFEM_BLOCK), 0, ctx->stream, A->n, A->ell_K, (const DiaOffsets*)A->dia_dev,
                     A->ell_bound_mode == 2 ? A->dia_flags : nullptr, A->ell_cols, A->ell_vals, d);
  MFEM_CHECK_LAUNCH();
  return MFEM_OK;
}

static std::atomic<int64_t> g_sym_launches{0};
extern "C" int64_t mfem_debug_sym_spmv_count(void) { return g_sym_launches; }
int mfem_spmv_ell_launch(mfem_context_s* ctx, mfem_csr_s* A, const double* vals, const double* x, double* y, double alpha, double beta,
                         const double* dotw, double* partials, int* n_partials, const int32_t* done_flag, const SpmvPart& part) {
  if (!A->ell_vals || vals != A->ell_src) return 0;
  int cap = ctx->num_cus * g_ell.grid_mult;
  if (cap > MFEM_MAX_PARTIALS) cap = MFEM_MAX_PARTIALS;
  if (part.part != 0) cap /= 2;
  if (part.part == 2) {
    int64_t rows = 0;
    for (int z = 0; z < part.nz; ++z) rows += part.hi[z] - part.lo[z];
    const int64_t want = rows / 512 + 2 * part.nz + 1;
    if (want < cap) cap = (int)want;
  }
  const SpmvArgs a{x, y, alpha, beta, dotw, partials, n_partials, done_flag, part};
  int rc = MFEM_OK;
  switch (A->ell_bound_mode == 2 ? A->dia_kernel : DIA_NONE) {
    case DIA_SYMP:
    case DIA_SYM27:
      if (part.part != 2) ++g_sym_launches;
      rc = mfem_sym_launch(ctx, A, (DiaKernel)A->dia_kernel, a);
      break;
    case DIA_ROWS_TRIPLES:
    case DIA_ROWS: rc = mfem_dia_launch(ctx, A, A->dia_kernel == DIA_ROWS_TRIPLES, cap, a); break;
    default: {
      const int grid = mfem_grid_for((A->n + 1) / 2, MFEM_BLOCK, cap);
      hipLaunchKernelGGL((k_spmv_ell<2, 1>), dim3(grid), dim3(MFEM_BLOCK), 0, ctx->stream, A->n, A->ell_npad, A->ell_K, A->ell_cols, A->ell_vals, x,
                         y, alpha, beta, dotw, partials, done_flag, part);
      MFEM_CHECK_LAUNCH();
      if (n_partials && partials) *n_partials = grid;
    }
  }
  return rc ? rc : 1;
}

int64_t mfem_ell_entries(const mfem_context_s* ctx, const mfem_csr_s* A, int32_t* sweep) {
  const DiaKernel k = mfem_dia_layout_planned(A) ? mfem_dia_kernel_wanted(A) : DIA_NONE;
  if (sweep) *sweep = k == DIA_SYMP ? 2 : k == DIA_SYM27 ? 1 : 0;
  return k == DIA_SYMP || k == DIA_SYM27 ? mfem_sym_entries(ctx, A, k) : (int64_t)A->ell_K * A->ell_npad;
}
int64_t mfem_ell_design_bytes(const mfem_context_s* ctx, const mfem_csr_s* A) {
  int32_t sym = 0;
  const int64_t ent = mfem_ell_entries(ctx, A, &sym);
  if (!mfem_dia_layout_planned(A)) return ent * 12 + A->n * 16;
  const int64_t reg = (int64_t)A->dia_regular_blocks * 128;
  int64_t b = ent * 8 + A->n * 16 + (A->n > reg ? A->n - reg : 0) * (int64_t)A->ell_K * 4;
  if (sym == 2) b += mfem_symp_steps(A) * (int64_t)sp_xn(mfem_symp_bands(A)) * 8 - mfem_symp_swept_rows(A) * 8;
  return b;
}
```

metafem.jl_amd/csrc/spmv_sym.hip:

```cpp
#include "blas1.h"
#include "spmv_ell.h"

#define SYM_ROWS 512
#define SYM_THREADS (SYM_ROWS / 2)
#define SYM_WG_PER_CU 3
__global__ __launch_bounds__(SYM_THREADS) void k_spmv_sym27(int64_t n, int64_t npad, int K, const DiaOffsets* __restrict__ Op,
                                                             const int32_t* __restrict__ flags, const int32_t* __restrict__ cols,
                                                             const double* __restrict__ vals, const double* __restrict__ x,
                                                             double* __restrict__ y, double alpha, double beta,
                                                             const double* __restrict__ dotw, double* __restrict__ partials,
                                                             const int32_t* __restrict__ done_flag, int64_t c0, int64_t c1, int S, int nsteps, int cls, int gs,
                                                             int part) {
  __shared__ __attribute__((aligned(16))) double hist[9][SYM_ROWS];
  __shared__ __attribute__((aligned(16))) double exch[4][SYM_ROWS];
  __shared__ double red[16];
  if (done_flag && done_flag[0]) return;
  const int32_t* off = Op->off[cls];
  const int tid = threadIdx.x;
  double dot_acc = 0.0;
  const int tile = blockIdx.x % S, seg = blockIdx.x / S;
  const int nseg = gs / S + (tile < gs % S ? 1 : 0);
  const int seg_len = part == 2 ? 0 : (nsteps + nseg - 1) / nseg;
  bool have_hist = false;
  e_d2 up_next[4] = {{0.0, 0.0}, {0.0, 0.0}, {0.0, 0.0}, {0.0, 0.0}};
  {
    const int64_t chunk = c0 + tile + (int64_t)S * ((int64_t)seg * seg_len);
    if (part != 2 && seg * seg_len < nsteps && chunk < c1) {
      const double* v = vals + ell_base(chunk * SYM_ROWS + 2 * tid, K);
#pragma unroll
      for (int u = 0; u < 4; ++u) up_next[u] = SYM_LD(reinterpret_cast<const e_d2*>(v + (14 + u) * ELL_B));
    }
  }
  for (int it = 0; it < seg_len; ++it) {
    const int step = seg * seg_len + it;
    const int64_t chunk = c0 + tile + (int64_t)S * step;
    if (step >= nsteps || chunk >= c1) break;
    const int64_t r = chunk * SYM_ROWS + 2 * tid;
    const double* v = vals + ell_base(r, K);
    e_d2 acc = {0.0, 0.0};
    e_d2 up[4];
#pragma unroll
    for (int u = 0; u < 4; ++u) {
      up[u] = up_next[u];
      *reinterpret_cast<e_d2*>(&exch[u][2 * tid]) = up[u];
    }
    __syncthreads();
    auto slot = [&](int s, const double* tab, int lp, bool ok) -> e_d2 {
      e_d2 w;
      if (ok && lp >= 0 && lp + 1 < SYM_ROWS) {
        w.x = tab[lp];
        w.y = tab[lp + 1];
      } else {
        w = SYM_LD(reinterpret_cast<const e_d2*>(v + s * ELL_B));
      }
      return w;
    };
#define SYM_RUN(va, vb, vc, s0)                                          \
  {                                                                      \
    const u_d2* xp = reinterpret_cast<const u_d2*>(x + r + off[s0]);     \
    const u_d2 xa = xp[0], xb = xp[1];                                   \
    acc.x += va.x != 0.0 ? va.x * xa.x : 0.0;                            \
    acc.y += va.y != 0.0 ? va.y * xa.y : 0.0;                            \
    acc.x += vb.x != 0.0 ? vb.x * xa.y : 0.0;                            \
    acc.y += vb.y != 0.0 ? vb.y * xb.x : 0.0;                            \
    acc.x += vc.x != 0.0 ? vc.x * xb.x : 0.0;                            \
    acc.y += vc.y != 0.0 ? vc.y * xb.y : 0.0;                            \
    if (s0 == 12) {                                                      \
      xself0 = xa.y;                                                     \
      xself1 = xb.x;                                                     \
    }                                                                    \
  }
    double xself0 = 0.0, xself1 = 0.0;
    const int lph = 2 * tid + S * SYM_ROWS;
#pragma unroll
    for (int s = 0; s < 9; s += 3) {
      const e_d2 va = slot(s, hist[8 - s], lph + off[s], have_hist);
      const e_d2 vb = slot(s + 1, hist[7 - s], lph + off[s + 1], have_hist);
      const e_d2 vc = slot(s + 2, hist[6 - s], lph + off[s + 2], have_hist);
      SYM_RUN(va, vb, vc, s);
    }
    {
      const e_d2 va = slot(9, exch[3], 2 * tid + off[9], true);
      const e_d2 vb = slot(10, exch[2], 2 * tid + off[10], true);
      const e_d2 vc = slot(11, exch[1], 2 * tid + off[11], true);
      SYM_RUN(va, vb, vc, 9);
    }
    {
      e_d2 va;
      va.y = up[0].x;
      if (tid > 0) va.x = exch[0][2 * tid - 1];
      else va.x = v[12 * ELL_B];
      const e_d2 vb = SYM_LD(reinterpret_cast<const e_d2*>(v + 13 * ELL_B));
      SYM_RUN(va, vb, up[0], 12);
    }
    SYM_RUN(up[1], up[2], up[3], 15);
    if (it + 1 < seg_len && step + 1 < nsteps && chunk + S < c1) {
      const double* vn = vals + ell_base((chunk + S) * SYM_ROWS + 2 * tid, K);
#pragma unroll
      for (int u = 0; u < 4; ++u) up_next[u] = SYM_LD(reinterpret_cast<const e_d2*>(vn + (14 + u) * ELL_B));
    }
    __syncthreads();
#pragma unroll
    for (int s = 18; s < 27; s += 3) {
      const e_d2 va = SYM_LD(reinterpret_cast<const e_d2*>(v + s * ELL_B));
      const e_d2 vb = SYM_LD(reinterpret_cast<const e_d2*>(v + (s + 1) * ELL_B));
      const e_d2 vc = SYM_LD(reinterpret_cast<const e_d2*>(v + (s + 2) * ELL_B));
      SYM_RUN(va, vb, vc, s);
      *reinterpret_cast<e_d2*>(&hist[s - 18][2 * tid]) = va;
      *reinterpret_cast<e_d2*>(&hist[s - 17][2 * tid]) = vb;
      *reinterpret_cast<e_d2*>(&hist[s - 16][2 * tid]) = vc;
    }
#undef SYM_RUN
    have_hist = true;
    double y0 = alpha * acc.x, y1 = alpha * acc.y;
    if (beta != 0.0) {
      y0 += beta * y[r];
      y1 += beta * y[r + 1];
    }
    y[r] = y0;
    y[r + 1] = y1;
    if (dotw) {
      if (dotw == x) dot_acc += y0 * xself0 + y1 * xself1;
      else dot_acc += y0 * dotw[r] + y1 * dotw[r + 1];
    }
  }
  if (part != 1) {
    const int64_t nchunks = (n + SYM_ROWS - 1) / SYM_ROWS;
    for (int64_t q = blockIdx.x;; q += gridDim.x) {
      const int64_t ch = q < c0 ? q : c1 + (q - c0);
      if (ch >= nchunks) break;
      const int64_t r = ch * SYM_ROWS + 2 * tid;
      if (r < n) dia_rows<2, 3, true>(r, n, npad, K, *Op, flags, cols, vals, x, y, alpha, beta, dotw, 0, dot_acc);
    }
  }
  if (partials) {
    const double b = block_reduce_sum(dot_acc, red);
    if (threadIdx.x == 0) partials[blockIdx.x] = b;
  }
}

__global__ __launch_bounds__(MFEM_BLOCK) void k_sym27_check(int K, const DiaOffsets* __restrict__ Op, const double* __restrict__ vals,
                                                              int64_t row_lo, int64_t row_hi, int cls, int32_t* __restrict__ bad) {
  const int32_t* off = Op->off[cls];
  const int64_t stride = (int64_t)gridDim.x * blockDim.x;
  int fail = 0;
  for (int64_t r = row_lo + blockIdx.x * (int64_t)blockDim.x + threadIdx.x; r < row_hi; r += stride) {
    const double* v = vals + ell_base(r, K);
    for (int s = 0; s < 13; ++s) {
      const int64_t rs = r + off[s];
      if (rs < row_lo) continue;
      const double a = v[s * ELL_B], b = vals[ell_base(rs, K) + (26 - s) * ELL_B];
      if (__double_as_longlong(a) != __double_as_longlong(b) && !(a == 0.0 && b == 0.0)) fail = 1;
    }
  }
  if (fail) atomicOr(bad, 1);
}


__constant__ int32_t c_sp_ecell[SP_BMAX][sp_epad(SP_BMAX)];
static int symp_upload_tables(int device) {
  static bool done[64] = {};
  if (device >= 0 && device < 64 && done[device]) return MFEM_OK;
  int32_t h[SP_BMAX][sp_epad(SP_BMAX)];
  for (int B = 1; B <= SP_BMAX; ++B)
    for (int e = 0; e < sp_epad(SP_BMAX); ++e) {
      int s_, l_, c_, cell = 0;
      h[B - 1][e] = sp_edge(e, s_, l_, c_, cell, B) ? cell : sp_tab(B);
    }
  MFEM_CHECK_HIP(hipMemcpyToSymbol(HIP_SYMBOL(c_sp_ecell), h, sizeof(h)));
  if (device >= 0 && device < 64) done[device] = true;
  return MFEM_OK;
}

__device__ __forceinline__ void symp_rim_unit(const SympGeom& Gm, const double* __restrict__ rimv, int64_t u, int lane, const double* __restrict__ x,
                                              double* __restrict__ y, double alpha, double beta, const double* __restrict__ dotw, double& dot_acc) {
  const int64_t g = u * SPT_UNIT + lane;
  if (g >= Gm.rim_rows) return;
  const int pl = (int)(g / Gm.rim_pp);
  int j = 0, k = 0;
  spt_rim_row((int)(g - (int64_t)pl * Gm.rim_pp), Gm.m2, Gm.ms1, Gm.ms2, j, k);
  const int64_t r = (int64_t)(Gm.p0 + pl) * Gm.PL + (int64_t)j * Gm.m2 + k;
  const double* v = rimv + u * SPT_UNIT_DOUBLES + lane;
  double vv[27], xv[27];
#pragma unroll
  for (int s = 0; s < 27; ++s) {
    vv[s] = SYM_LD(v + s * SPT_UNIT);
    int64_t idx = r + (int64_t)(s / 9 - 1) * Gm.PL + (int64_t)(sp_dj(s) * Gm.m2 + sp_dk(s));
    idx = idx < 0 ? 0 : idx;
    xv[s] = x[idx < Gm.nx ? idx : Gm.nx - 1];
  }
  double acc = 0.0;
#pragma unroll
  for (int s = 0; s < 27; ++s) acc += vv[s] != 0.0 ? vv[s] * xv[s] : 0.0;
  double y0 = alpha * acc;
  if (beta != 0.0) y0 += beta * y[r];
  y[r] = y0;
  if (dotw) dot_acc += y0 * dotw[r];
}
__global__ __launch_bounds__(64) void k_symp_rim(SympGeom Gm, const double* __restrict__ rimv, const double* __restrict__ x, double* __restrict__ y,
                                                  double alpha, double beta, const double* __restrict__ dotw, double* __restrict__ partials,
                                                  const int32_t* __restrict__ done_flag) {
  if (done_flag && done_flag[0]) return;
  double dot_acc = 0.0;
  for (int64_t u = blockIdx.x; u < Gm.rim_units; u += gridDim.x) symp_rim_unit(Gm, rimv, u, threadIdx.x, x, y, alpha, beta, dotw, dot_acc);
  if (partials) {
    const double w = wave_reduce_sum(dot_acc);
    if (threadIdx.x == 0) partials[blockIdx.x] = w;
  }
}

template <int MODE, int B, int DC, int CS>
__device__ __forceinline__ void symp_sweep(const SympGeom& Gm, const double* __restrict__ pv, const double* __restrict__ x,
                                           double* __restrict__ y, double alpha, double beta,
                                           const double* __restrict__ dotw, double* __restrict__ partials,
                                           const int32_t* __restrict__ done_flag, int32_t* __restrict__ bad, const SympTail& tail, const SympConst& cst,
                                           const uint32_t* __restrict__ sflags) {
  static_assert(CS == 0 || MODE == 0, "the check pass reads the stored copy");
  constexpr int XL = sp_xl(B), XN = sp_xn(B), XU = sp_xu(B), NE = sp_ne(B), EU = sp_eu(B), MAINB = sp_main(B, DC), LOWB = sp_low(B);
  constexpr int NSL = sp_nslots(DC), S0 = 27 - NSL;
  constexpr int BM = NSL * SP_ROWS, BL = 13 * SP_ROWS, BT = SP_L * SP_LS;
  __shared__ __attribute__((aligned(16))) double xs[3][XL][SP_XW];
  __shared__ __attribute__((aligned(16))) double tab[sp_tab(B) + 2 + (CS ? 28 : 0)];
  double* const ctab = tab + sp_tab(B) + 2;
  if (done_flag && done_flag[0]) return;
  const int lane = threadIdx.x, lj = lane / SP_PW, pk = lane % SP_PW, lb0 = lj * SP_LS + 2 * pk;
  const int NP = Gm.NR * Gm.NPk, nplanes = Gm.p1 - Gm.p0;
  const int xcd = blockIdx.x & 7, pc = NP / 8, prem = NP % 8, pcnt = pc + (xcd < prem ? 1 : 0), pfirst = xcd * pc + (xcd < prem ? xcd : prem);
  int ecell[EU];
#pragma unroll
  for (int u = 0; u < EU; ++u) ecell[u] = c_sp_ecell[B - 1][lane + 64 * u];
  if (CS && lane == 0) {
#pragma unroll
    for (int s = 0; s < 27; ++s) ctab[s] = cst.v[s];
  }
  int fw = 0;
  int64_t ft0 = 0;
  int cur_patch = -1, bp = 0, bc = 1, bn = 2;
  int nb = 1;
  bool have_hist = false;
  bool vxb[B], vyb[B];
  int64_t rin = 0;
  int xo[XU], xa[XU];
  double dot_acc = 0.0;
  int fail = 0;
  e_d2 cur[B][NSL];
  int cdc[B];
  e_d2 keep[3];
  double ed[EU], xr[XU];
  auto xidx = [&](int plane, int u) -> int64_t {
    int64_t idx = (int64_t)plane * Gm.PL + xo[u];
    idx = idx < 0 ? 0 : idx;
    return idx < Gm.nx ? idx : Gm.nx - 1;
  };
  auto request = [&](const double* v, int b, bool fl) {
    if (CS && fl) return;
    if (vxb[b]) {
#pragma unroll
      for (int u = 0; u < NSL; ++u) cur[b][u] = SYM_LD(reinterpret_cast<const e_d2*>(v + b * BM + 2 * lane + u * SP_ROWS));
      if (DC && MODE == 0) cdc[b] = SYM_LD(reinterpret_cast<const unsigned short*>(v + sp_coff(B, DC)) + b * (SP_ROWS / 2) + lane);
    } else {
#pragma unroll
      for (int u = 0; u < NSL; ++u) cur[b][u] = (e_d2){0.0, 0.0};
      if (DC) cdc[b] = 0;
    }
  };
  auto request_step = [&](const double* v, int pnext, bool fl) {
    if (MODE == 0) {
      if (!(CS && fl)) {
#pragma unroll
        for (int u = 0; u < EU - 1; ++u) ed[u] = SYM_LD(v + B * BM + lane + 64 * u);
        ed[EU - 1] = lane < NE - 64 * (EU - 1) ? SYM_LD(v + B * BM + lane + 64 * (EU - 1)) : 0.0;
      }
#pragma unroll
      for (int u = 0; u < XU - 1; ++u) xr[u] = x[xidx(pnext, u)];
      xr[XU - 1] = lane < XN - 64 * (XU - 1) ? x[xidx(pnext, XU - 1)] : 0.0;
    }
  };
  auto stage_x = [&](int buf, int plane) {
    double* dst = &xs[buf][0][0];
#pragma unroll
    for (int u = 0; u < XU - 1; ++u) dst[xa[u]] = x[xidx(plane, u)];
    if (lane < XN - 64 * (XU - 1)) dst[xa[XU - 1]] = x[xidx(plane, XU - 1)];
  };
  const int W = gridDim.x >> 3, jw = blockIdx.x >> 3, rot = spc_rot(Gm.NPk);
  for (int rk = 0; W * rk < pcnt * Gm.nseg; ++rk) {
  const int run = spc_run(W, jw, rk, rot);
  if (run >= pcnt * Gm.nseg) continue;
  const int patch = pfirst + run % pcnt, seg = run / pcnt;
  const int64_t t0 = (int64_t)patch * nplanes + (int64_t)nplanes * seg / Gm.nseg, t1 = (int64_t)patch * nplanes + (int64_t)nplanes * (seg + 1) / Gm.nseg;
  cur_patch = -1;
  for (int64_t t = t0; t < t1; ++t) {
    const int p = Gm.p0 + (int)(t - (int64_t)patch * nplanes);
    const int64_t step = (int64_t)(p - Gm.p0) * NP + patch;
    const double* v = pv + step * MAINB;
    const double* vlow = pv + (int64_t)NP * nplanes * MAINB + step * LOWB;
    const bool more = t + 1 < t1 && p + 1 < Gm.p1;
    if (CS && (patch != cur_patch || t - ft0 >= 63)) {
      ft0 = t;
      const int64_t tl = t + lane, sl = (tl - (int64_t)patch * nplanes) * NP + patch;
      fw = tl < t1 ? (int)((sflags[sl >> 2] >> (8 * (int)(sl & 3))) & 255u) : 0;
    }
    const bool fnow = CS && __builtin_amdgcn_readlane(fw, (int)(t - ft0)) != 0;
    const bool fnext = CS && more && __builtin_amdgcn_readlane(fw, (int)(t + 1 - ft0)) != 0;
    if (patch != cur_patch) {
      cur_patch = patch;
      const int j0 = (patch / Gm.NPk) * (SP_L * B), k0 = (patch % Gm.NPk) * SP_W;
      const int k = k0 + 2 * pk;
      nb = 1;
#pragma unroll
      for (int b = 0; b < B; ++b) {
        const int j = j0 + SP_L * b + lj;
        vxb[b] = j < Gm.m1 && k < Gm.m2;
        vyb[b] = j < Gm.m1 && k + 1 < Gm.m2;
        if (b > 0 && j0 + SP_L * b < Gm.m1) nb = b + 1;
      }
      rin = (int64_t)(j0 + lj) * Gm.m2 + k;
#pragma unroll
      for (int u = 0; u < XU; ++u) {
        const int tt = lane + 64 * u, xl = tt / SP_XC, xc = tt - SP_XC * xl;
        xo[u] = (j0 - 1 + xl) * Gm.m2 + (k0 - 1 + xc);
        xa[u] = xl * SP_XW + xc;
      }
      have_hist = false;
      __syncthreads();
#pragma unroll
      for (int b = 0; b < B; ++b)
        if (b < nb) request(v, b, fnow);
      request_step(v, p + 1, fnow);
      if (MODE == 0) {
        stage_x(bp, p - 1);
        stage_x(bc, p);
#pragma unroll
        for (int b = 0; b < B; ++b) {
          if (b < nb && !fnow) {
#pragma unroll
            for (int s = 0; s < 9; ++s) {
              const e_d2 w = vxb[b] ? SYM_LD(reinterpret_cast<const e_d2*>(vlow + b * BL + 2 * lane + s * SP_ROWS)) : (e_d2){0.0, 0.0};
              double* c = tab + sp_tbase(s, B) + (sp_dj(s) + sp_adj(s)) * SP_LS + sp_dk(s) + 2 + b * BT + lb0;
              c[0] = w.x;
              c[1] = w.y;
            }
          }
        }
      }
    }
    if (CS && fnow) {
      {
        double* dst = &xs[bn][0][0];
#pragma unroll
        for (int u = 0; u < XU - 1; ++u) dst[xa[u]] = xr[u];
        if (lane < XN - 64 * (XU - 1)) dst[xa[XU - 1]] = xr[XU - 1];
      }
      __syncthreads();
      if (more && fnext) request_step(v + (int64_t)NP * MAINB, p + 2, true);
#pragma unroll
      for (int b = 0; b < B; ++b) {
        e_d2 acc = {0.0, 0.0};
        double xself0 = 0.0, xself1 = 0.0;
        auto crun = [&](int s, int buf, int dj, bool self) {
#pragma clang fp contract(off)
          const double* xp = &xs[buf][SP_L * b + lj + 1 + dj][2 * pk];
          const e_d2 xa2 = *reinterpret_cast<const e_d2*>(xp), xb2 = *reinterpret_cast<const e_d2*>(xp + 2);
          const double c0 = ctab[s], c1 = ctab[s + 1], c2 = ctab[s + 2];
          acc.x = acc.x + c0 * xa2.x;
          acc.y = acc.y + c0 * xa2.y;
          acc.x = acc.x + c1 * xa2.y;
          acc.y = acc.y + c1 * xb2.x;
          acc.x = acc.x + c2 * xb2.x;
          acc.y = acc.y + c2 * xb2.y;
          if (self) {
            xself0 = xa2.y;
            xself1 = xb2.x;
          }
        };
        crun(0, bp, -1, false);
        crun(3, bp, 0, false);
        crun(6, bp, 1, false);
        crun(9, bc, -1, false);
        crun(12, bc, 0, true);
        crun(15, bc, 1, false);
        crun(18, bn, -1, false);
        crun(21, bn, 0, false);
        crun(24, bn, 1, false);
        const int64_t r = (int64_t)p * Gm.PL + rin + (int64_t)(SP_L * b) * Gm.m2;
        double y0 = alpha * acc.x, y1 = alpha * acc.y;
        if (beta != 0.0) {
          y0 += beta * y[r];
          y1 += beta * y[r + 1];
        }
        __builtin_nontemporal_store((u_d2){y0, y1}, reinterpret_cast<u_d2*>(y + r));
        if (dotw) {
          if (dotw == x) {
            dot_acc += y0 * xself0;
            dot_acc += y1 * xself1;
          } else {
            dot_acc += y0 * dotw[r];
            dot_acc += y1 * dotw[r + 1];
          }
        }
      }
      __syncthreads();
      const int b_ = bp;
      bp = bc;
      bc = bn;
      bn = b_;
      if (!(more && fnext)) cur_patch = -1;
      continue;
    }
#pragma unroll
    for (int b = 0; b < B; ++b) {
    if (b < nb) {
    const int lb = lb0 + b * BT;
    const bool vx = vxb[b], vy = vyb[b], lastb = b + 1 >= nb;
#pragma unroll
    for (int s = 9; s < 13; ++s) *reinterpret_cast<e_d2*>(tab + sp_tbase(s, B) + sp_adj(s) * SP_LS + 2 + lb) = cur[b][26 - s - S0];
    e_d2 low[13];
    if (MODE == 0) {
      if (b == 0) {
#pragma unroll
        for (int u = 0; u < EU; ++u) tab[ecell[u]] = ed[u];
        double* dst = &xs[bn][0][0];
#pragma unroll
        for (int u = 0; u < XU - 1; ++u) dst[xa[u]] = xr[u];
        if (lane < XN - 64 * (XU - 1)) dst[xa[XU - 1]] = xr[XU - 1];
      }
    } else {
#pragma unroll
      for (int s = 0; s < 13; ++s) low[s] = vx ? SYM_LD(reinterpret_cast<const e_d2*>(vlow + b * BL + 2 * lane + s * SP_ROWS)) : (e_d2){0.0, 0.0};
    }
    e_d2 mine[NSL];
#pragma unroll
    for (int u = 0; u < NSL; ++u) mine[u] = cur[b][u];
    const int mcd = DC && MODE == 0 ? cdc[b] : 0;
    __syncthreads();
    if (more) {
      request(v + (int64_t)NP * MAINB, b, fnext);
      if (lastb) request_step(v + (int64_t)NP * MAINB, p + 2, fnext);
    }
    auto mirrored = [&](int s) -> e_d2 {
      const double* c = tab + sp_tbase(s, B) + (sp_dj(s) + sp_adj(s)) * SP_LS + sp_dk(s) + 2 + lb;
      e_d2 w;
      w.x = c[0];
      w.y = c[1];
      return w;
    };
    e_d2 acc = {0.0, 0.0};
    double xself0 = 0.0, xself1 = 0.0;
    auto run = [&](const e_d2& va, const e_d2& vb, const e_d2& vc, int buf, int dj, bool self) {
#pragma clang fp contract(off)
      const double* xp = &xs[buf][SP_L * b + lj + 1 + dj][2 * pk];
      const e_d2 xa2 = *reinterpret_cast<const e_d2*>(xp), xb2 = *reinterpret_cast<const e_d2*>(xp + 2);
      acc.x = acc.x + va.x * xa2.x;
      acc.y = acc.y + va.y * xa2.y;
      acc.x = acc.x + vb.x * xa2.y;
      acc.y = acc.y + vb.y * xb2.x;
      acc.x = acc.x + vc.x * xb2.x;
      acc.y = acc.y + vc.y * xb2.y;
      if (self) {
        xself0 = xa2.y;
        xself1 = xb2.x;
      }
    };
    if (MODE == 1) {
#pragma unroll
      for (int s = 0; s < 13; ++s) {
        const int dj = sp_dj(s), dk = sp_dk(s), gl = SP_L * b + lj;
        const bool in = gl + dj >= 0 && gl + dj < SP_L * nb && (dk < 0 ? pk > 0 : dk > 0 ? pk < SP_PW - 1 : true);
        if (in && vx && (s >= 9 || have_hist)) {
          const e_d2 m = mirrored(s);
          if (__double_as_longlong(m.x) != __double_as_longlong(low[s].x) && !(m.x == 0.0 && low[s].x == 0.0)) fail = 1;
          if (vy && __double_as_longlong(m.y) != __double_as_longlong(low[s].y) && !(m.y == 0.0 && low[s].y == 0.0)) fail = 1;
        }
      }
    } else {
      run(mirrored(0), mirrored(1), mirrored(2), bp, -1, false);
      run(mirrored(3), mirrored(4), mirrored(5), bp, 0, false);
      run(mirrored(6), mirrored(7), mirrored(8), bp, 1, false);
      run(mirrored(9), mirrored(10), mirrored(11), bc, -1, false);
      e_d2 dg;
      if (DC) {
        dg.x = __longlong_as_double(Gm.unit + (long long)(signed char)(mcd & 255));
        dg.y = __longlong_as_double(Gm.unit + (long long)(signed char)((mcd >> 8) & 255));
      } else {
        dg = mine[0];
      }
      run(mirrored(12), dg, mine[14 - S0], bc, 0, true);
      run(mine[15 - S0], mine[16 - S0], mine[17 - S0], bc, 1, false);
    }
    __syncthreads();
#pragma unroll
    for (int s = 3; s < 9; ++s) *reinterpret_cast<e_d2*>(tab + sp_tbase(s, B) + sp_adj(s) * SP_LS + 2 + lb) = mine[26 - s - S0];
    if (B > 1 && !lastb) {
#pragma unroll
      for (int s = 0; s < 3; ++s) keep[s] = mine[26 - s - S0];
    } else {
#pragma unroll
      for (int s = 0; s < 3; ++s) {
        *reinterpret_cast<e_d2*>(tab + sp_tbase(s, B) + sp_adj(s) * SP_LS + 2 + lb) = mine[26 - s - S0];
        if (B > 1 && b > 0) *reinterpret_cast<e_d2*>(tab + sp_tbase(s, B) + sp_adj(s) * SP_LS + 2 + lb - BT) = keep[s];
      }
    }
    if (MODE == 0) {
      run(mine[18 - S0], mine[19 - S0], mine[20 - S0], bn, -1, false);
      run(mine[21 - S0], mine[22 - S0], mine[23 - S0], bn, 0, false);
      run(mine[24 - S0], mine[25 - S0], mine[26 - S0], bn, 1, false);
      const int64_t r = (int64_t)p * Gm.PL + rin + (int64_t)(SP_L * b) * Gm.m2;
      double y0 = alpha * acc.x, y1 = alpha * acc.y;
      if (beta != 0.0) {
        if (vx) y0 += beta * y[r];
        if (vy) y1 += beta * y[r + 1];
      }
      {
        if (vy) __builtin_nontemporal_store((u_d2){y0, y1}, reinterpret_cast<u_d2*>(y + r));
        else if (vx) __builtin_nontemporal_store(y0, y + r);
      }
      if (dotw) {
        if (dotw == x) {
          if (vx) dot_acc += y0 * xself0;
          if (vy) dot_acc += y1 * xself1;
        } else {
          if (vx) dot_acc += y0 * dotw[r];
          if (vy) dot_acc += y1 * dotw[r + 1];
        }
      }
    }
    }
    }
    have_hist = true;
    if (MODE == 0) {
      const int b_ = bp;
      bp = bc;
      bc = bn;
      bn = b_;
    }
    if (!more) cur_patch = -1;
  }
  }
  if (MODE == 0 && tail.on) {
    const int64_t UA = (tail.lo + 127) / 128, ub = tail.hi / 128, UB = (tail.n + 127) / 128 - ub;
    for (int64_t u = blockIdx.x; u < UA + UB; u += gridDim.x) {
      const int64_t r = (u < UA ? u : ub + (u - UA)) * 128 + 2 * lane;
      if (r < tail.n)
        dia_rows<2, 3, true>(r, tail.n, tail.npad, tail.K, *tail.Op, tail.flags, tail.cols, tail.ell, x, y, alpha, beta, dotw, 0, dot_acc,
                             tail.lo, tail.hi);
    }
  }
  if (MODE == 0 && tail.rim) {
    const double* rimv = pv + (int64_t)NP * nplanes * (MAINB + LOWB);
    for (int64_t u = blockIdx.x; u < Gm.rim_units; u += gridDim.x) symp_rim_unit(Gm, rimv, u, lane, x, y, alpha, beta, dotw, dot_acc);
  }
  if (MODE == 1) {
    if (fail) atomicOr(bad, 1);
  } else if (partials) {
    const double w = wave_reduce_sum(dot_acc);
    if (lane == 0) partials[blockIdx.x] = w;
  }
}

template <int MODE, int B, int DC>
__global__ __launch_bounds__(64) void k_spmv_symp(SympGeom Gm, const double* __restrict__ pv, const double* __restrict__ x,
                                                   double* __restrict__ y, double alpha, double beta,
                                                   const double* __restrict__ dotw, double* __restrict__ partials,
                                                   const int32_t* __restrict__ done_flag, int32_t* __restrict__ bad, SympTail tail) {
  symp_sweep<MODE, B, DC, 0>(Gm, pv, x, y, alpha, beta, dotw, partials, done_flag, bad, tail, SympConst{}, nullptr);
}
template <int B, int DC>
__global__ __launch_bounds__(64) void k_spmv_symp_const(SympGeom Gm, const double* __restrict__ pv, const double* __restrict__ x,
                                                         double* __restrict__ y, double alpha, double beta,
                                                         const double* __restrict__ dotw, double* __restrict__ partials,
                                                         const int32_t* __restrict__ done_flag, SympTail tail, SympConst cst,
                                                         const uint32_t* __restrict__ sflags) {
  symp_sweep<0, B, DC, 1>(Gm, pv, x, y, alpha, beta, dotw, partials, done_flag, nullptr, tail, cst, sflags);
}

__global__ __launch_bounds__(MFEM_BLOCK) void k_symp_bind(SympGeom Gm, int K, const double* __restrict__ ell, double* __restrict__ pv) {
  const int lane = threadIdx.x & 63, lj = lane / SP_PW, pk = lane % SP_PW;
  const int NP = Gm.NR * Gm.NPk, B = Gm.B;
  const int MAINB = sp_main(B), LOWB = sp_low(B), NEB = sp_ne(B), EPADB = sp_epad(B);
  const int64_t T = (int64_t)NP * (Gm.p1 - Gm.p0);
  for (int64_t t = (int64_t)blockIdx.x * (MFEM_BLOCK / 64) + (threadIdx.x >> 6); t < T; t += (int64_t)gridDim.x * (MFEM_BLOCK / 64)) {
    const int nplanes = Gm.p1 - Gm.p0, patch = (int)(t / nplanes), p = Gm.p0 + (int)(t % nplanes);
    const int j0 = (patch / Gm.NPk) * (SP_L * B), k0 = (patch % Gm.NPk) * SP_W;
    const int64_t step = (int64_t)(p - Gm.p0) * NP + patch;
    double* out = pv + step * MAINB;
    double* outlow = pv + T * MAINB + step * LOWB;
    for (int b = 0; b < B; ++b) {
      const int j = j0 + SP_L * b + lj, k = k0 + 2 * pk;
      const bool vx = j < Gm.m1 && k < Gm.m2, vy = j < Gm.m1 && k + 1 < Gm.m2;
      const int64_t r = (int64_t)p * Gm.PL + (int64_t)j * Gm.m2 + k;
      const int64_t b0 = ell_base(r, K), b1 = ell_base(r + 1, K);
      for (int s0 = 0; s0 < 27; s0 += 9) {
        e_d2 w[9];
#pragma unroll
        for (int u = 0; u < 9; ++u) {
          w[u].x = vx ? ell[b0 + (s0 + u) * ELL_B] : 0.0;
          w[u].y = vy ? ell[b1 + (s0 + u) * ELL_B] : 0.0;
        }
#pragma unroll
        for (int u = 0; u < 9; ++u) {
          const int sl = s0 + u;
          double* dst = sl < 13 ? outlow + b * 13 * SP_ROWS + sl * SP_ROWS : out + b * 14 * SP_ROWS + (sl - 13) * SP_ROWS;
          *reinterpret_cast<e_d2*>(dst + 2 * lane) = w[u];
        }
      }
    }
    for (int e = lane; e < EPADB; e += 64) {
      int s = 0, line = 0, col = 0, cell = 0;
      double val = 0.0;
      if (e < NEB && sp_edge(e, s, line, col, cell, B) && j0 + line < Gm.m1 && k0 + col < Gm.m2)
        val = ell[ell_base((int64_t)p * Gm.PL + (int64_t)(j0 + line) * Gm.m2 + k0 + col, K) + s * ELL_B];
      out[B * 14 * SP_ROWS + e] = val;
    }
  }
}

static void sym27_plan(mfem_csr_s* A, const int32_t* off, int lc, int64_t PL, int64_t run_lo, int64_t run_hi) {
  const int64_t Sc = (PL + SYM_ROWS / 2) / SYM_ROWS;
  if (Sc < 8 || Sc > MFEM_MAX_PARTIALS / 2) return;
  const int64_t bpc = SYM_ROWS / ELL_B, c0 = (run_lo + bpc - 1) / bpc, c1 = run_hi / bpc;
  if (c1 - c0 < 4 * Sc) return;
  int64_t mx = 0, myz = 0;
  for (int t = 0; t < SYM_ROWS / 2; ++t) {
    for (int q = 0; q < 9; ++q) {
      const int64_t lp = 2 * t + Sc * SYM_ROWS + off[q];
      if (lp >= 0 && lp + 1 < SYM_ROWS) mx += 2;
    }
    for (int q = 9; q < 12; ++q) {
      const int64_t lp = 2 * t + off[q];
      if (lp >= 0 && lp + 1 < SYM_ROWS) myz += 2;
    }
    myz += t > 0 ? 2 : 1;
  }
  if (20 * (mx + myz) < 5 * 13 * SYM_ROWS) return;
  A->sym_state = 1;
  A->sym_c0 = c0;
  A->sym_c1 = c1;
  A->sym_S = (int)Sc;
  A->sym_cls = lc;
  A->sym_mx = mx;
  A->sym_myz = myz;
}
static void symp_plan(mfem_csr_s* A, int lc, int64_t m2, int64_t PL, int64_t run_lo, int64_t run_hi) {
  A->symp_state = -1;
  if (PL % m2 != 0 || PL / m2 < 2 || PL >= (int64_t)1 << 30) return;
  const int64_t p0 = (run_lo * ELL_B + PL - 1) / PL, p1 = run_hi * ELL_B / PL;
  if (p1 - p0 < 4 || p0 < 1) return;
  A->symp_state = 1;
  A->symp_m2 = (int)m2;
  A->symp_m1 = (int)(PL / m2);
  A->symp_PL = PL;
  A->symp_p0 = (int)p0;
  A->symp_p1 = (int)p1;
  A->symp_NS = (A->symp_m1 + SP_L - 1) / SP_L;
  A->symp_NPk = (A->symp_m2 + SP_W - 1) / SP_W;
  A->sym_cls = lc;
}
void mfem_sym_plan(mfem_csr_s* A, const int32_t* off, int lc, int64_t m2, int64_t PL, int64_t run_lo, int64_t run_hi) {
  sym27_plan(A, off, lc, PL, run_lo, run_hi);
  symp_plan(A, lc, m2, PL, run_lo, run_hi);
}

bool mfem_sym_wanted(const mfem_csr_s* A, DiaKernel k) {
  if (!g_ell.sym || !A->dia_triples) return false;
  const bool all = g_layout_min_rows_dia == 0;
  if (k == DIA_SYM27) return A->sym_state == 1 && (all || A->sym_c1 - A->sym_c0 >= 2700);
  return A->symp_state == 1 && g_ell.symp && (all || (int64_t)(A->symp_p1 - A->symp_p0) * A->symp_PL >= 24000000 || A->symp_m2 > 256);
}

static int sym27_grid(const mfem_context_s* ctx, const mfem_csr_s* A, int64_t* nsteps_out) {
  const int64_t nsteps = (A->sym_c1 - A->sym_c0 + A->sym_S - 1) / A->sym_S;
  const int resident = SYM_WG_PER_CU * ctx->num_cus;
  int nseg = resident / A->sym_S;
  if (nseg < 1) nseg = 1;
  if ((int64_t)A->sym_S * nseg * 10 < (int64_t)resident * 8) nseg = (8 * ctx->num_cus + A->sym_S - 1) / A->sym_S;
  while (nseg > 1 && (int64_t)A->sym_S * nseg > MFEM_MAX_PARTIALS - 512) --nseg;
  if (nseg > nsteps / 8) nseg = (int)(nsteps / 8);
  if (nseg < 1) nseg = 1;
  if (nsteps_out) *nsteps_out = nsteps;
  return A->sym_S * nseg;
}
struct SympExt { int ms1, ms2, NS, NPk, NR; };
static SympExt symp_ext(const mfem_csr_s* A, int B, int trim) {
  SympExt e;
  e.ms1 = spt_ms1(A->symp_m1, B, trim != 0);
  e.ms2 = spt_ms2(A->symp_m2, trim != 0);
  e.NS = (e.ms1 + SP_L - 1) / SP_L;
  e.NPk = spt_cols(e.ms2);
  e.NR = spt_rows(e.ms1, B);
  return e;
}
static SympExt symp_ext(const mfem_csr_s* A) { return symp_ext(A, mfem_symp_bands(A), mfem_symp_trim(A)); }
static int symp_nseg(const mfem_context_s* ctx, const mfem_csr_s* A) {
  const SympExt e = symp_ext(A);
  return spt_nseg((int64_t)e.NR * e.NPk, (int64_t)sp_wg_per_cu(mfem_symp_bands(A)) * ctx->num_cus, A->symp_p1 - A->symp_p0);
}
SympGeom mfem_symp_geom(const mfem_context_s* ctx, const mfem_csr_s* A) {
  const int B = mfem_symp_bands(A);
  const SympExt e = symp_ext(A);
  SympGeom G{A->symp_PL, A->n, A->symp_m1, A->symp_m2, A->symp_p0, A->symp_p1, e.NS, e.NPk, symp_nseg(ctx, A), B, e.NR, A->symp_DC, sp_unit_bits(A->symp_dneg)};
  G.ms1 = e.ms1;
  G.ms2 = e.ms2;
  G.rim_pp = spt_rim(G.m1, G.m2, G.ms1, G.ms2);
  G.rim_rows = (int64_t)G.rim_pp * (G.p1 - G.p0);
  G.rim_units = spt_units(G.rim_rows);
  return G;
}
int64_t mfem_symp_steps(const mfem_csr_s* A, int B, int trim) {
  if (B < 1) B = mfem_symp_bands(A);
  const SympExt e = symp_ext(A, B, trim < 0 ? mfem_symp_trim(A) : trim);
  return (int64_t)e.NR * e.NPk * (A->symp_p1 - A->symp_p0);
}
int64_t mfem_symp_copy_doubles(const mfem_csr_s* A, int B, int trim) {
  const SympExt e = symp_ext(A, B, trim);
  return mfem_symp_steps(A, B, trim) * sp_step(B) + spt_units((int64_t)spt_rim(A->symp_m1, A->symp_m2, e.ms1, e.ms2) * (A->symp_p1 - A->symp_p0)) * SPT_UNIT_DOUBLES +
         spc_flag_doubles(mfem_symp_steps(A, B, trim));
}
unsigned char* mfem_symp_flags_of(double* pvals, const SympGeom& G) {
  return (unsigned char*)(pvals + (int64_t)G.NR * G.NPk * (G.p1 - G.p0) * sp_step(G.B, G.DC) + G.rim_units * SPT_UNIT_DOUBLES);
}
int64_t mfem_symp_swept_rows(const mfem_csr_s* A) {
  const SympExt e = symp_ext(A);
  return (int64_t)(A->symp_p1 - A->symp_p0) * e.ms1 * e.ms2;
}
#define SYMP_RIM_GRID 256
static int symp_grid(const mfem_context_s* ctx, const mfem_csr_s* A) {
  const int B = mfem_symp_bands(A);
  const SympExt e = symp_ext(A);
  const int64_t NP = (int64_t)e.NR * e.NPk;
  int64_t g = 8 * ((NP + 7) / 8) * symp_nseg(ctx, A);
  int64_t cap = (int64_t)sp_wg_per_cu(B) * ctx->num_cus;
  if (cap > MFEM_MAX_PARTIALS - 1024 - SYMP_RIM_GRID) cap = MFEM_MAX_PARTIALS - 1024 - SYMP_RIM_GRID;
  cap &= ~(int64_t)7;
  if (g > cap) g = cap;
  return g < 8 ? 8 : (int)g;
}

int64_t mfem_sym_entries(const mfem_context_s* ctx, const mfem_csr_s* A, DiaKernel k) {
  if (k == DIA_SYM27) {
    const int64_t nch = A->sym_c1 - A->sym_c0;
    return (int64_t)A->ell_K * A->ell_npad - ((nch - sym27_grid(ctx, A, nullptr)) * A->sym_mx + nch * A->sym_myz);
  }
  const int B = mfem_symp_bands(A);
  const SympExt x = symp_ext(A);
  const int NP = x.NR * x.NPk, nplanes = A->symp_p1 - A->symp_p0, nseg = symp_nseg(ctx, A);
  int64_t e = (int64_t)A->ell_K * (A->ell_npad - (int64_t)nplanes * A->symp_PL), codes = 0;
  e += 27 * (int64_t)spt_rim(A->symp_m1, A->symp_m2, x.ms1, x.ms2) * nplanes;
  for (int patch = 0; patch < NP; ++patch) {
    int64_t nv = 0;
    for (int lp = 0; lp < 64 * B; ++lp) {
      const int j = (patch / x.NPk) * (SP_L * B) + lp / SP_PW, kk = (patch % x.NPk) * SP_W + 2 * (lp % SP_PW);
      if (j < A->symp_m1 && kk < A->symp_m2) ++nv;
    }
    e += (28 * nv + sp_ne(B)) * nplanes + 18 * nv * nseg;
    codes += 2 * nv * nplanes;
  }
  if (A->symp_vals ? A->symp_CS : A->symp_cs_last) {
    const int64_t fl = A->symp_vals ? A->symp_flagged : A->symp_flagged_last;
    e -= fl * spc_saved_entries(B) - spc_flag_doubles((int64_t)NP * nplanes);
    codes -= fl * spc_saved_codes(B);
  }
  if (mfem_symp_coded(A)) e -= codes - (codes + 7) / 8;
  return e;
}

static auto symp_const_kernel(const SympGeom& G) {
  if (G.DC) return G.B == 2 ? k_spmv_symp_const<2, 1> : k_spmv_symp_const<1, 1>;
  return G.B == 2 ? k_spmv_symp_const<2, 0> : k_spmv_symp_const<1, 0>;
}
template <int MODE>
static auto symp_kernel(const SympGeom& G) {
  if (G.DC) return G.B == 2 ? k_spmv_symp<MODE, 2, 1> : k_spmv_symp<MODE, 1, 1>;
  return G.B == 2 ? k_spmv_symp<MODE, 2, 0> : k_spmv_symp<MODE, 1, 0>;
}

static std::atomic<long long> g_symp_fp_checks{0};
extern "C" long long mfem_debug_symp_fingerprint_count(void) { return g_symp_fp_checks; }

int mfem_sym_verdict(mfem_context_s* ctx, mfem_csr_s* A, DiaKernel k, const double* buf, double* pvals, const SympGeom& G, bool direct, bool fp_made, bool* ok,
                     bool* dc_refused, int* dneg, bool flags_made, SympConst* cst, int64_t* flagged) {
  int32_t* d_bad = ctx->d_flags + 9;
  const size_t fp_ints = flags_made && k == DIA_SYMP ? MFEM_NFLAGS - 16 : 4;
  auto read_const = [&]() {
    if (!(flags_made && k == DIA_SYMP && cst && flagged)) return;
    *flagged = ctx->h_flags[SPC_COUNT_AT];
    memcpy(cst, ctx->h_flags + SPC_REF_AT, sizeof(SympConst));
  };
  *dc_refused = false;
  *dneg = 0;
  if (k == DIA_SYMP) {
    { const int rt = symp_upload_tables(ctx->device); if (rt) return rt; }
    if (!direct) {
      const int64_t T = mfem_symp_steps(A);
      const int gb = (int)(T / 4 + 1 < (int64_t)ctx->num_cus * 32 ? T / 4 + 1 : (int64_t)ctx->num_cus * 32);
      hipLaunchKernelGGL(k_symp_bind, dim3(gb), dim3(MFEM_BLOCK), 0, ctx->stream, G, A->ell_K, buf, pvals);
      MFEM_CHECK_LAUNCH();
    }
    if (fp_made) {
      MFEM_CHECK_HIP(hipMemcpyAsync(ctx->h_flags + 16, ctx->d_flags + 16, fp_ints * sizeof(int32_t), hipMemcpyDeviceToHost, ctx->stream));
      MFEM_CHECK_HIP(hipStreamSynchronize(ctx->stream));
      unsigned long long fpv;
      memcpy(&fpv, ctx->h_flags + 16, sizeof(fpv));
      *ok = fpv == 0;
      *dc_refused = G.DC && ctx->h_flags[18] != 0;
      *dneg = G.DC && ctx->h_flags[19] != 0;
      read_const();
      ++g_symp_fp_checks;
      return MFEM_OK;
    }
  }
  MFEM_CHECK_HIP(hipMemsetAsync(d_bad, 0, sizeof(int32_t), ctx->stream));
  if (k == DIA_SYMP)
    hipLaunchKernelGGL(symp_kernel<1>(G), dim3(symp_grid(ctx, A)), dim3(64), 0, ctx->stream, G, (const double*)pvals,
                       (const double*)nullptr, (double*)nullptr, 0.0, 0.0, (const double*)nullptr, (double*)nullptr, (const int32_t*)nullptr, d_bad,
                       SympTail{});
  else
    hipLaunchKernelGGL(k_sym27_check, dim3(ctx->num_cus * 8), dim3(MFEM_BLOCK), 0, ctx->stream, A->ell_K, (const DiaOffsets*)A->dia_dev, buf,
                       A->sym_c0 * SYM_ROWS, A->sym_c1 * SYM_ROWS, A->sym_cls, d_bad);
  MFEM_CHECK_LAUNCH();
  MFEM_CHECK_HIP(hipMemcpyAsync(ctx->h_flags + 9, d_bad, sizeof(int32_t), hipMemcpyDeviceToHost, ctx->stream));
  if (k == DIA_SYMP && (G.DC || flags_made)) MFEM_CHECK_HIP(hipMemcpyAsync(ctx->h_flags + 18, ctx->d_flags + 18, (fp_ints - 2) * sizeof(int32_t), hipMemcpyDeviceToHost, ctx->stream));
  MFEM_CHECK_HIP(hipStreamSynchronize(ctx->stream));
  *ok = ctx->h_flags[9] == 0;
  *dc_refused = k == DIA_SYMP && G.DC && ctx->h_flags[18] != 0;
  *dneg = k == DIA_SYMP && G.DC && ctx->h_flags[19] != 0;
  read_const();
  return MFEM_OK;
}

int mfem_sym_launch(mfem_context_s* ctx, mfem_csr_s* A, DiaKernel k, const SpmvArgs& a) {
  const DiaOffsets* O = (const DiaOffsets*)A->dia_dev;
  int np = 0;
  if (k == DIA_SYM27) {
    int64_t nsteps = 0;
    const int gs = sym27_grid(ctx, A, &nsteps);
    const int64_t outside = (A->n + SYM_ROWS - 1) / SYM_ROWS - (A->sym_c1 - A->sym_c0);
    np = a.part.part == 2 ? (int)(outside < 1 ? 1 : outside < 512 ? outside : 512) : gs;
    hipLaunchKernelGGL(k_spmv_sym27, dim3(np), dim3(SYM_THREADS), 0, ctx->stream, A->n, A->ell_npad, A->ell_K, O, A->dia_flags, A->ell_cols, A->ell_vals,
                       a.x, a.y, a.alpha, a.beta, a.dotw, a.partials, a.done_flag, A->sym_c0, A->sym_c1, A->sym_S, (int)nsteps, A->sym_cls, gs, a.part.part);
    MFEM_CHECK_LAUNCH();
  } else {
    const SympGeom G = mfem_symp_geom(ctx, A);
    const int64_t lo = (int64_t)G.p0 * G.PL, hi = (int64_t)G.p1 * G.PL;
    SympTail tl{};
    if (a.part.part == 0 && g_ell.symp_tail) tl = SympTail{1, A->ell_K, G.rim_units > 0, A->n, A->ell_npad, lo, hi, O, A->dia_flags, A->ell_cols, A->ell_vals};
    if (a.part.part != 2) {
      np = symp_grid(ctx, A);
      if (A->symp_CS) {
        SympConst cst{};
        memcpy(cst.v, A->symp_cst, sizeof(cst.v));
        cst.code = A->symp_ccode;
        cst.valid = 1;
        hipLaunchKernelGGL(symp_const_kernel(G), dim3(np), dim3(64), 0, ctx->stream, G, (const double*)A->symp_vals, a.x, a.y, a.alpha, a.beta, a.dotw,
                           a.partials, a.done_flag, tl, cst, (const uint32_t*)mfem_symp_flags_of(A->symp_vals, G));
      } else {
        hipLaunchKernelGGL(symp_kernel<0>(G), dim3(np), dim3(64), 0, ctx->stream, G, (const double*)A->symp_vals, a.x, a.y, a.alpha, a.beta, a.dotw,
                           a.partials, a.done_flag, (int32_t*)nullptr, tl);
      }
      MFEM_CHECK_LAUNCH();
    }
    if (a.part.part == 2 || (a.part.part == 0 && !tl.on)) {
      int go = 0;
      const int rc = mfem_dia_launch_outside(ctx, A, a, a.partials ? a.partials + np : nullptr, lo, hi, &go);
      if (rc) return rc;
      np += go;
      if (G.rim_units > 0) {
        const int gr = (int)(G.rim_units < SYMP_RIM_GRID ? G.rim_units : SYMP_RIM_GRID);
        hipLaunchKernelGGL(k_symp_rim, dim3(gr), dim3(64), 0, ctx->stream, G, (const double*)A->symp_vals + (int64_t)G.NR * G.NPk * (G.p1 - G.p0) * sp_step(G.B, G.DC),
                           a.x, a.y, a.alpha, a.beta, a.dotw, a.partials ? a.partials + np : nullptr, a.done_flag);
        MFEM_CHECK_LAUNCH();
        np += gr;
      }
    }
  }
  if (a.n_partials && a.partials) *a.n_partials = np;
  return MFEM_OK;
}
```

Measured before the change: 34.00 billion DOF-updates/s.

## Add cost-balanced device-built schedule for symmetric patch SpMV sweep

Replaces the static even split of patches across XCDs and waves with a schedule table built once on the device. A prefix sum of per-plane-block costs, weighted by flagged vs unflagged planes and start-up cost, sets balanced chain boundaries. Dot-product partials are now written per plane into a sums buffer, reduced with DPP-based wave sums and folded by a separate kernel, and the tail/rim work is given its own partial slots. This aims to remove load imbalance across workgroups, at the cost of an extra fold kernel launch, extra memory traffic for per-plane sums, and a one-time scheduling kernel per bind.

```diff
diff --git a/include/metafem_mi355x_debug.h b/include/metafem_mi355x_debug.h
--- a/include/metafem_mi355x_debug.h
+++ b/include/metafem_mi355x_debug.h
@@ -13,6 +13,7 @@
 long long mfem_debug_symp_trim_count(void);
 long long mfem_debug_symp_const_count(void);
 long long mfem_debug_symp_const_steps(void);
+int mfem_debug_symp_sched(int64_t* info, int32_t* table, int64_t cap);
 int mfem_debug_spmv_scaled_layout(mfem_context ctx, mfem_csr A, const double* vals, const double* ssym, const double* x, double* y, double alpha, double beta,
                                   const double* dotw, double* partials_out , int32_t cap, int32_t* n_partials , int32_t* form );
 int mfem_debug_set(const char* key, int64_t a, int64_t b);
diff --git a/metafem.jl_amd/_lib.py b/metafem.jl_amd/_lib.py
--- a/metafem.jl_amd/_lib.py
+++ b/metafem.jl_amd/_lib.py
@@ -174,6 +174,7 @@
     "mfem_debug_symp_trim_count": (C.c_longlong, []),
     "mfem_debug_symp_const_count": (C.c_longlong, []),
     "mfem_debug_symp_const_steps": (C.c_longlong, []),
+    "mfem_debug_symp_sched": (c_int, [C.POINTER(c_int64), C.POINTER(c_int32), c_int64]),
     "mfem_debug_spmv_scaled_layout": (c_int, [P, P, P, P, P, P, c_double, c_double, P, P, c_int32, C.POINTER(c_int32), C.POINTER(c_int32)]),
     "mfem_debug_set": (c_int, [C.c_char_p, c_int64, c_int64]),
     "mfem_debug_graph_comm_count": (c_int, []),
diff --git a/metafem.jl_amd/csrc/api.hip b/metafem.jl_amd/csrc/api.hip
--- a/metafem.jl_amd/csrc/api.hip
+++ b/metafem.jl_amd/csrc/api.hip
@@ -327,6 +327,7 @@
 int mfem_debug_set_remainder(int);
 int mfem_debug_set_recheck_scale(double);
 int mfem_debug_set_bsell(int);
+int mfem_debug_set_symp_sched(int64_t, int64_t);
 }
 extern int g_mesh_gather_rows, g_mesh_abl, g_mesh_stage_min_itp, g_mesh_term_matrix;
 extern int g_op_wave_forms, g_op_wave_min_itp;
@@ -358,6 +359,7 @@
   if (k == "remainder") return mfem_debug_set_remainder((int)a);
   if (k == "mesh_gather_rows") { g_mesh_gather_rows = (int)a; return MFEM_OK; }
   if (k == "bsell") return mfem_debug_set_bsell((int)a);
+  if (k == "symp_sched") return mfem_debug_set_symp_sched(a, b);
   if (k == "op_wave_forms") { g_op_wave_forms = (int)a; g_op_wave_min_itp = b > 0 ? (int)b : 10; return MFEM_OK; }
   if (k == "mesh_stage_min_itp") { g_mesh_stage_min_itp = a > 0 ? (int)a : 16; return MFEM_OK; }
   if (k == "mesh_term_matrix") { g_mesh_term_matrix = (int)a; return MFEM_OK; }
diff --git a/metafem.jl_amd/csrc/common.h b/metafem.jl_amd/csrc/common.h
--- a/metafem.jl_amd/csrc/common.h
+++ b/metafem.jl_amd/csrc/common.h
@@ -169,6 +169,7 @@
   int symp_trim;
   int symp_DC;
   int symp_dneg;
+  int symp_sW;
   int symp_CS;
   int symp_cs_last;
   int64_t symp_flagged, symp_flagged_last;
diff --git a/metafem.jl_amd/csrc/spmv_ell.h b/metafem.jl_amd/csrc/spmv_ell.h
--- a/metafem.jl_amd/csrc/spmv_ell.h
+++ b/metafem.jl_amd/csrc/spmv_ell.h
@@ -5,6 +5,7 @@
 #include "spmv_symp.h"
 #include "symp_trim_decide.h"
 #include "symp_const_decide.h"
+#include "symp_sched_decide.h"
 
 #define ELL_B 128
 __host__ __device__ __forceinline__ int64_t ell_base(int64_t r, int K) { return (r >> 7) * ((int64_t)K * ELL_B) + (r & (ELL_B - 1)); }
@@ -47,6 +48,12 @@
   const int32_t* flags;
   const int32_t* cols;
   const double* ell;
+};
+
+struct SympSched {
+  const int32_t* tab;
+  double* sums;
+  int vg;
 };
 
 #if defined(DV_ABL) && DV_ABL == 1
@@ -206,4 +213,5 @@
 int mfem_sym_verdict(mfem_context_s* ctx, mfem_csr_s* A, DiaKernel k, const double* buf, double* pvals, const SympGeom& G, bool direct, bool fp_made, bool* ok,
                      bool* dc_refused, int* dneg, bool flags_made = false, SympConst* cst = nullptr, int64_t* flagged = nullptr);
 unsigned char* mfem_symp_flags_of(double* pvals, const SympGeom& G);
+int mfem_symp_schedule(mfem_context_s* ctx, mfem_csr_s* A, const SympGeom& G, double* pvals, bool use_flags);
 int mfem_sym_launch(mfem_context_s* ctx, mfem_csr_s* A, DiaKernel k, const SpmvArgs& a);
diff --git a/metafem.jl_amd/csrc/spmv_ell.hip b/metafem.jl_amd/csrc/spmv_ell.hip
--- a/metafem.jl_amd/csrc/spmv_ell.hip
+++ b/metafem.jl_amd/csrc/spmv_ell.hip
@@ -331,6 +331,8 @@
     A->symp_dc_last = A->symp_DC;
     if (A->symp_DC) ++g_symp_coded_binds;
     if (G.rim_units > 0) ++g_symp_trim_binds;
+    rc = mfem_symp_schedule(ctx, A, mfem_symp_geom(ctx, A), pvals, A->symp_CS != 0);
+    if (rc) return rc;
   }
   return MFEM_OK;
 }
@@ -359,7 +361,7 @@
   A->ell_bound_mode = A->dia_kernel = DIA_NONE;
   A->ell_vals = A->symp_vals = nullptr;
   A->ell_src = nullptr;
-  A->symp_B = A->symp_DC = A->symp_dneg = A->symp_trim = A->symp_CS = 0;
+  A->symp_B = A->symp_DC = A->symp_dneg = A->symp_trim = A->symp_CS = A->symp_sW = 0;
   A->symp_flagged = 0;
 }
 void mfem_ell_free(mfem_csr_s* A) {
diff --git a/metafem.jl_amd/csrc/spmv_sym.hip b/metafem.jl_amd/csrc/spmv_sym.hip
--- a/metafem.jl_amd/csrc/spmv_sym.hip
+++ b/metafem.jl_amd/csrc/spmv_sym.hip
@@ -209,12 +209,29 @@
   }
 }
 
+template <int CTRL>
+__device__ __forceinline__ double symp_dpp(double v) {
+  const int lo = __builtin_amdgcn_update_dpp(0, __double2loint(v), CTRL, 0xF, 0xF, true);
+  const int hi = __builtin_amdgcn_update_dpp(0, __double2hiint(v), CTRL, 0xF, 0xF, true);
+  return __hiloint2double(hi, lo);
+}
+__device__ __forceinline__ double symp_lane(double v, int l) {
+  return __hiloint2double(__builtin_amdgcn_readlane(__double2hiint(v), l), __builtin_amdgcn_readlane(__double2loint(v), l));
+}
+__device__ __forceinline__ double symp_wave_sum(double v) {
+  v += symp_dpp<0xB1>(v);
+  v += symp_dpp<0x4E>(v);
+  v += symp_dpp<0x141>(v);
+  v += symp_dpp<0x140>(v);
+  return ((symp_lane(v, 0) + symp_lane(v, 16)) + symp_lane(v, 32)) + symp_lane(v, 48);
+}
+
 template <int MODE, int B, int DC, int CS>
 __device__ __forceinline__ void symp_sweep(const SympGeom& Gm, const double* __restrict__ pv, const double* __restrict__ x,
                                            double* __restrict__ y, double alpha, double beta,
                                            const double* __restrict__ dotw, double* __restrict__ partials,
                                            const int32_t* __restrict__ done_flag, int32_t* __restrict__ bad, const SympTail& tail, const SympConst& cst,
-                                           const uint32_t* __restrict__ sflags) {
+                                           const uint32_t* __restrict__ sflags, const SympSched& sc) {
   static_assert(CS == 0 || MODE == 0, "the check pass reads the stored copy");
   constexpr int XL = sp_xl(B), XN = sp_xn(B), XU = sp_xu(B), NE = sp_ne(B), EU = sp_eu(B), MAINB = sp_main(B, DC), LOWB = sp_low(B);
   constexpr int NSL = sp_nslots(DC), S0 = 27 - NSL;
@@ -225,7 +242,7 @@
   if (done_flag && done_flag[0]) return;
   const int lane = threadIdx.x, lj = lane / SP_PW, pk = lane % SP_PW, lb0 = lj * SP_LS + 2 * pk;
   const int NP = Gm.NR * Gm.NPk, nplanes = Gm.p1 - Gm.p0;
-  const int xcd = blockIdx.x & 7, pc = NP / 8, prem = NP % 8, pcnt = pc + (xcd < prem ? 1 : 0), pfirst = xcd * pc + (xcd < prem ? xcd : prem);
+  const int xcd = blockIdx.x & 7, pfirst = sc.tab[xcd], pcnt = sc.tab[xcd + 1] - pfirst, W = sc.tab[10], NR = sc.tab[11], SL = sc.tab[12], NBP = sps_nbp(nplanes, SL);
   int ecell[EU];
 #pragma unroll
   for (int u = 0; u < EU; ++u) ecell[u] = c_sp_ecell[B - 1][lane + 64 * u];
@@ -242,6 +259,15 @@
   int64_t rin = 0;
   int xo[XU], xa[XU];
   double dot_acc = 0.0;
+  constexpr bool LATE = CS == 0, EVERY = CS == 1 && B == 1;
+  double pend = 0.0;
+  int64_t pend_t = -1;
+  auto flush_sum = [&]() {
+    if (pend_t >= 0) {
+      if (lane == 0) sc.sums[pend_t] = pend;
+      pend_t = -1;
+    }
+  };
   int fail = 0;
   e_d2 cur[B][NSL];
   int cdc[B];
@@ -282,12 +308,20 @@
     for (int u = 0; u < XU - 1; ++u) dst[xa[u]] = x[xidx(plane, u)];
     if (lane < XN - 64 * (XU - 1)) dst[xa[XU - 1]] = x[xidx(plane, XU - 1)];
   };
-  const int W = gridDim.x >> 3, jw = blockIdx.x >> 3, rot = spc_rot(Gm.NPk);
-  for (int rk = 0; W * rk < pcnt * Gm.nseg; ++rk) {
-  const int run = spc_run(W, jw, rk, rot);
-  if (run >= pcnt * Gm.nseg) continue;
-  const int patch = pfirst + run % pcnt, seg = run / pcnt;
-  const int64_t t0 = (int64_t)patch * nplanes + (int64_t)nplanes * seg / Gm.nseg, t1 = (int64_t)patch * nplanes + (int64_t)nplanes * (seg + 1) / Gm.nseg;
+  const int jw = blockIdx.x >> 3;
+  for (int rk = 0; rk < NR && jw < W; ++rk) {
+  const int32_t* chain = sc.tab + SPS_HEAD + 2 * ((xcd * NR + rk) * W + jw);
+  if (chain[0] >= chain[1]) continue;
+  const int seg = sps_seg_of(NBP, Gm.nseg, pcnt, chain[0]);
+  const int sb0 = sps_seg_b0(NBP, Gm.nseg, seg), nbs = sps_seg_b0(NBP, Gm.nseg, seg + 1) - sb0;
+  int q = chain[0] - pcnt * sb0;
+  const int q1 = chain[1] - pcnt * sb0;
+  while (q < q1) {
+  const int pi = q / nbs, bi = q - pi * nbs, patch = pfirst + pi;
+  const int qe = (pi + 1) * nbs < q1 ? (pi + 1) * nbs : q1;
+  const int pl0 = (sb0 + bi) * SL, pl1 = (sb0 + bi + (qe - q)) * SL < nplanes ? (sb0 + bi + (qe - q)) * SL : nplanes;
+  const int64_t t0 = (int64_t)patch * nplanes + pl0, t1 = (int64_t)patch * nplanes + pl1;
+  q = qe;
   cur_patch = -1;
   for (int64_t t = t0; t < t1; ++t) {
     const int p = Gm.p0 + (int)(t - (int64_t)patch * nplanes);
@@ -405,6 +439,14 @@
       bc = bn;
       bn = b_;
       if (!(more && fnext)) cur_patch = -1;
+      if (EVERY) {
+        sc.sums[t] = symp_wave_sum(dot_acc);
+        dot_acc = 0.0;
+      } else if (partials) {
+        const double w = symp_wave_sum(dot_acc);
+        if (lane == 0) sc.sums[t] = w;
+        dot_acc = 0.0;
+      }
       continue;
     }
 #pragma unroll
@@ -433,6 +475,7 @@
     for (int u = 0; u < NSL; ++u) mine[u] = cur[b][u];
     const int mcd = DC && MODE == 0 ? cdc[b] : 0;
     __syncthreads();
+    if (MODE == 0 && LATE && b == 0) flush_sum();
     if (more) {
       request(v + (int64_t)NP * MAINB, b, fnext);
       if (lastb) request_step(v + (int64_t)NP * MAINB, p + 2, fnext);
@@ -534,43 +577,140 @@
       bn = b_;
     }
     if (!more) cur_patch = -1;
-  }
-  }
-  if (MODE == 0 && tail.on) {
-    const int64_t UA = (tail.lo + 127) / 128, ub = tail.hi / 128, UB = (tail.n + 127) / 128 - ub;
-    for (int64_t u = blockIdx.x; u < UA + UB; u += gridDim.x) {
-      const int64_t r = (u < UA ? u : ub + (u - UA)) * 128 + 2 * lane;
-      if (r < tail.n)
-        dia_rows<2, 3, true>(r, tail.n, tail.npad, tail.K, *tail.Op, tail.flags, tail.cols, tail.ell, x, y, alpha, beta, dotw, 0, dot_acc,
-                             tail.lo, tail.hi);
-    }
-  }
-  if (MODE == 0 && tail.rim) {
-    const double* rimv = pv + (int64_t)NP * nplanes * (MAINB + LOWB);
-    for (int64_t u = blockIdx.x; u < Gm.rim_units; u += gridDim.x) symp_rim_unit(Gm, rimv, u, lane, x, y, alpha, beta, dotw, dot_acc);
-  }
-  if (MODE == 1) {
-    if (fail) atomicOr(bad, 1);
-  } else if (partials) {
-    const double w = wave_reduce_sum(dot_acc);
-    if (lane == 0) partials[blockIdx.x] = w;
-  }
+    if (MODE == 0 && EVERY) {
+      sc.sums[t] = symp_wave_sum(dot_acc);
+      dot_acc = 0.0;
+    } else if (MODE == 0 && !LATE && partials) {
+      const double w = symp_wave_sum(dot_acc);
+      if (lane == 0) sc.sums[t] = w;
+      dot_acc = 0.0;
+    } else if (MODE == 0 && partials) {
+      pend = symp_wave_sum(dot_acc);
+      pend_t = t;
+      dot_acc = 0.0;
+    }
+  }
+  if (MODE == 0 && LATE) flush_sum();
+  }
+  }
+  if (MODE == 0) {
+    for (int vs = blockIdx.x; vs < sc.vg; vs += gridDim.x) {
+      dot_acc = 0.0;
+      if (tail.on) {
+        const int64_t UA = (tail.lo + 127) / 128, ub = tail.hi / 128, UB = (tail.n + 127) / 128 - ub;
+        for (int64_t u = vs; u < UA + UB; u += sc.vg) {
+          const int64_t r = (u < UA ? u : ub + (u - UA)) * 128 + 2 * lane;
+          if (r < tail.n)
+            dia_rows<2, 3, true>(r, tail.n, tail.npad, tail.K, *tail.Op, tail.flags, tail.cols, tail.ell, x, y, alpha, beta, dotw, 0, dot_acc,
+                                 tail.lo, tail.hi);
+        }
+      }
+      if (tail.rim) {
+        const double* rimv = pv + (int64_t)NP * nplanes * (MAINB + LOWB);
+        for (int64_t u = vs; u < Gm.rim_units; u += sc.vg) symp_rim_unit(Gm, rimv, u, lane, x, y, alpha, beta, dotw, dot_acc);
+      }
+      if (partials) {
+        const double w = wave_reduce_sum(dot_acc);
+        if (lane == 0) partials[sps_groups(NP) + vs] = w;
+      }
+    }
+  }
+  if (MODE == 1 && fail) atomicOr(bad, 1);
 }
 
 template <int MODE, int B, int DC>
 __global__ __launch_bounds__(64) void k_spmv_symp(SympGeom Gm, const double* __restrict__ pv, const double* __restrict__ x,
                                                    double* __restrict__ y, double alpha, double beta,
                                                    const double* __restrict__ dotw, double* __restrict__ partials,
-                                                   const int32_t* __restrict__ done_flag, int32_t* __restrict__ bad, SympTail tail) {
-  symp_sweep<MODE, B, DC, 0>(Gm, pv, x, y, alpha, beta, dotw, partials, done_flag, bad, tail, SympConst{}, nullptr);
+                                                   const int32_t* __restrict__ done_flag, int32_t* __restrict__ bad, SympTail tail, SympSched sc) {
+  symp_sweep<MODE, B, DC, 0>(Gm, pv, x, y, alpha, beta, dotw, partials, done_flag, bad, tail, SympConst{}, nullptr, sc);
 }
 template <int B, int DC>
 __global__ __launch_bounds__(64) void k_spmv_symp_const(SympGeom Gm, const double* __restrict__ pv, const double* __restrict__ x,
                                                          double* __restrict__ y, double alpha, double beta,
                                                          const double* __restrict__ dotw, double* __restrict__ partials,
                                                          const int32_t* __restrict__ done_flag, SympTail tail, SympConst cst,
-                                                         const uint32_t* __restrict__ sflags) {
-  symp_sweep<0, B, DC, 1>(Gm, pv, x, y, alpha, beta, dotw, partials, done_flag, nullptr, tail, cst, sflags);
+                                                         const uint32_t* __restrict__ sflags, SympSched sc) {
+  symp_sweep<0, B, DC, 1>(Gm, pv, x, y, alpha, beta, dotw, partials, done_flag, nullptr, tail, cst, sflags, sc);
+}
+
+#define SYMP_FOLD_WAVES 4
+__global__ __launch_bounds__(64 * SYMP_FOLD_WAVES) void k_symp_fold(int NP, int nplanes, const double* __restrict__ sums, double* __restrict__ partials,
+                                                                     const int32_t* __restrict__ done_flag) {
+  if (done_flag && done_flag[0]) return;
+  const int lane = threadIdx.x & 63, gi = blockIdx.x * SYMP_FOLD_WAVES + (threadIdx.x >> 6);
+  if (gi >= sps_groups(NP)) return;
+  double s = 0.0;
+  for (int patch = sps_fold_lo(NP, gi); patch < sps_fold_lo(NP, gi + 1); ++patch) {
+    const double* v = sums + (int64_t)patch * nplanes;
+    double a = 0.0;
+    for (int i = lane; i < nplanes; i += 64) a += v[i];
+    s += symp_wave_sum(a);
+  }
+  if (lane == 0) partials[gi] = s;
+}
+
+#define SPS_THREADS 1024
+__device__ __forceinline__ void sps_scan(int64_t* a, int64_t n, int64_t* sh) {
+  const int tid = threadIdx.x;
+  const int64_t chunk = (n + SPS_THREADS - 1) / SPS_THREADS, lo = tid * chunk < n ? tid * chunk : n, hi = lo + chunk < n ? lo + chunk : n;
+  int64_t s = 0;
+  for (int64_t i = lo; i < hi; ++i) s += a[i];
+  sh[tid] = s;
+  __syncthreads();
+  for (int d = 1; d < SPS_THREADS; d <<= 1) {
+    const int64_t t = tid >= d ? sh[tid - d] : 0;
+    __syncthreads();
+    sh[tid] += t;
+    __syncthreads();
+  }
+  s = tid > 0 ? sh[tid - 1] : 0;
+  for (int64_t i = lo; i < hi; ++i) {
+    s += a[i];
+    a[i] = s;
+  }
+  __syncthreads();
+}
+__global__ __launch_bounds__(SPS_THREADS) void k_symp_sched(SpsGeom g, const unsigned char* __restrict__ flags, int32_t* tab, int64_t* pb, int64_t* pp) {
+  __shared__ int64_t sh[SPS_THREADS];
+  const int tid = threadIdx.x, NBP = sps_nbp(g.nplanes, g.L);
+  for (int seg = 0; seg < g.nseg; ++seg) {
+    const int b0 = sps_seg_b0(NBP, g.nseg, seg), nbs = sps_seg_b0(NBP, g.nseg, seg + 1) - b0;
+    const int64_t off = sps_seg_off(g, seg);
+    for (int64_t r = tid; r < (int64_t)g.NP * nbs; r += SPS_THREADS) {
+      const int patch = (int)(r % g.NP), bi = (int)(r / g.NP);
+      pb[off + (int64_t)patch * nbs + bi] = sps_block_cost(g, flags, patch, b0 + bi, bi == 0);
+    }
+  }
+  __syncthreads();
+  sps_scan(pb, sps_blocks(g), sh);
+  for (int patch = tid; patch < g.NP; patch += SPS_THREADS) {
+    int64_t c = 0;
+    for (int seg = 0; seg < g.nseg; ++seg) {
+      const int nbs = sps_seg_b0(NBP, g.nseg, seg + 1) - sps_seg_b0(NBP, g.nseg, seg);
+      const int64_t a = sps_seg_off(g, seg) + (int64_t)patch * nbs;
+      if (nbs > 0) c += pb[a + nbs - 1] - (a > 0 ? pb[a - 1] : 0);
+    }
+    pp[patch] = c;
+  }
+  __syncthreads();
+  sps_scan(pp, g.NP, sh);
+  if (tid <= 8) tab[tid] = sps_xcd_bound(pp, g.NP, tid);
+  if (tid == 9) tab[9] = (int32_t)sps_blocks(g);
+  if (tid == 10) tab[10] = g.W;
+  if (tid == 11) tab[11] = g.R;
+  if (tid == 12) tab[12] = g.L;
+  if (tid == 13) tab[13] = g.nseg;
+  if (tid == 14) tab[14] = g.runs;
+  if (tid == 15) tab[15] = 0;
+  __syncthreads();
+  for (int64_t c = tid; c < sps_chains(g); c += SPS_THREADS) {
+    const int jw = (int)(c % g.W), rk = (int)((c / g.W) % g.R), xcd = (int)(c / ((int64_t)g.W * g.R));
+    int q0 = 0, q1 = 0;
+    sps_chain(g, pb, tab[xcd], tab[xcd + 1], rk, jw, q0, q1);
+    tab[sps_chain_at(g, xcd, rk, jw)] = q0;
+    tab[sps_chain_at(g, xcd, rk, jw) + 1] = q1;
+  }
 }
 
 __global__ __launch_bounds__(MFEM_BLOCK) void k_symp_bind(SympGeom Gm, int K, const double* __restrict__ ell, double* __restrict__ pv) {
@@ -710,30 +850,125 @@
   const SympExt e = symp_ext(A, B, trim < 0 ? mfem_symp_trim(A) : trim);
   return (int64_t)e.NR * e.NPk * (A->symp_p1 - A->symp_p0);
 }
+#define SYMP_RIM_GRID 256
+#define SYMP_MAX_GRID (MFEM_MAX_PARTIALS - 1024 - SYMP_RIM_GRID - SPS_MAX_GROUPS)
+static_assert(SYMP_MAX_GRID % 8 == 0 && SYMP_MAX_GRID >= 8 * 7 * 32, "every resident slot of the one-band sweep on 256 CUs");
+static int64_t symp_table_doubles() { return (SPS_HEAD + 2 * (int64_t)64 * SYMP_MAX_GRID + 1) / 2; }
 int64_t mfem_symp_copy_doubles(const mfem_csr_s* A, int B, int trim) {
   const SympExt e = symp_ext(A, B, trim);
-  return mfem_symp_steps(A, B, trim) * sp_step(B) + spt_units((int64_t)spt_rim(A->symp_m1, A->symp_m2, e.ms1, e.ms2) * (A->symp_p1 - A->symp_p0)) * SPT_UNIT_DOUBLES +
-         spc_flag_doubles(mfem_symp_steps(A, B, trim));
+  const int64_t steps = mfem_symp_steps(A, B, trim);
+  return steps * sp_step(B) + spt_units((int64_t)spt_rim(A->symp_m1, A->symp_m2, e.ms1, e.ms2) * (A->symp_p1 - A->symp_p0)) * SPT_UNIT_DOUBLES +
+         spc_flag_doubles(steps) + symp_table_doubles() + 2 * steps + (int64_t)e.NR * e.NPk;
 }
 unsigned char* mfem_symp_flags_of(double* pvals, const SympGeom& G) {
   return (unsigned char*)(pvals + (int64_t)G.NR * G.NPk * (G.p1 - G.p0) * sp_step(G.B, G.DC) + G.rim_units * SPT_UNIT_DOUBLES);
+}
+static int32_t* symp_table_of(double* pvals, const SympGeom& G) {
+  return (int32_t*)((double*)mfem_symp_flags_of(pvals, G) + spc_flag_doubles((int64_t)G.NR * G.NPk * (G.p1 - G.p0)));
+}
+static double* symp_sums_of(double* pvals, const SympGeom& G) { return (double*)symp_table_of(pvals, G) + symp_table_doubles(); }
+
+static std::atomic<int> g_sps_planes{0}, g_sps_record{0}, g_sps_nostart{0}, g_sps_len{0}, g_sps_div{1}, g_sps_ratio{0};
+extern "C" int mfem_debug_set_symp_sched(int64_t a, int64_t b) {
+  g_sps_planes = (int)(a & 1);
+  g_sps_record = (int)((a >> 1) & 1);
+  g_sps_nostart = (int)((a >> 2) & 1);
+  g_sps_len = (int)((a >> 8) & 255);
+  g_sps_div = (int)((a >> 16) & 255) > 1 ? (int)((a >> 16) & 255) : 1;
+  g_sps_ratio = b > 0 && b < 100000000 ? (int)b : 0;
+  return MFEM_OK;
 }
 int64_t mfem_symp_swept_rows(const mfem_csr_s* A) {
   const SympExt e = symp_ext(A);
   return (int64_t)(A->symp_p1 - A->symp_p0) * e.ms1 * e.ms2;
 }
-#define SYMP_RIM_GRID 256
-static int symp_grid(const mfem_context_s* ctx, const mfem_csr_s* A) {
+static int symp_grid(const mfem_context_s* ctx, const mfem_csr_s* A, bool whole = false) {
   const int B = mfem_symp_bands(A);
   const SympExt e = symp_ext(A);
-  const int64_t NP = (int64_t)e.NR * e.NPk;
-  int64_t g = 8 * ((NP + 7) / 8) * symp_nseg(ctx, A);
+  const int nseg = symp_nseg(ctx, A), NBP = sps_nbp(A->symp_p1 - A->symp_p0, SPS_PLANES);
+  int64_t g = 8 * (((int64_t)e.NR * e.NPk + 7) / 8) * ((NBP + nseg - 1) / nseg);
   int64_t cap = (int64_t)sp_wg_per_cu(B) * ctx->num_cus;
-  if (cap > MFEM_MAX_PARTIALS - 1024 - SYMP_RIM_GRID) cap = MFEM_MAX_PARTIALS - 1024 - SYMP_RIM_GRID;
+  if (cap > SYMP_MAX_GRID) cap = SYMP_MAX_GRID;
   cap &= ~(int64_t)7;
   if (g > cap) g = cap;
+  if (g < 8) g = 8;
+  if (!whole) g = (g / g_sps_div) & ~(int64_t)7;
   return g < 8 ? 8 : (int)g;
 }
+static SpsGeom symp_sps_geom(const mfem_context_s* ctx, const mfem_csr_s* A, const SympGeom& G, bool use_flags) {
+  SpsGeom g{};
+  g.NP = G.NR * G.NPk;
+  g.nplanes = G.p1 - G.p0;
+  g.nseg = G.nseg;
+  g.W = symp_grid(ctx, A) / 8;
+  g.L = sps_len(g_sps_len, g.NP, g.nplanes, g.nseg, g.W);
+  g.runs = !use_flags || g_sps_planes;
+  g.R = sps_rounds(g.NP, g.nseg, g.W, g.runs);
+  if (g.runs && sps_table_ints(g) > 2 * symp_table_doubles()) {
+    g.runs = 0;
+    g.R = g.nseg;
+  }
+  sps_costs(g, g_sps_ratio, g_sps_planes);
+  if (g_sps_nostart) g.su = g.sf = 0;
+  return g;
+}
+static std::vector<int32_t> g_sps_tab;
+static std::vector<int64_t> g_sps_pb;
+static SpsGeom g_sps_geom{};
+int mfem_symp_schedule(mfem_context_s* ctx, mfem_csr_s* A, const SympGeom& G, double* pvals, bool use_flags) {
+  const SpsGeom g = symp_sps_geom(ctx, A, G, use_flags);
+  const int64_t steps = (int64_t)g.NP * g.nplanes;
+  MFEM_REQUIRE(sps_table_ints(g) <= 2 * symp_table_doubles() && sps_blocks(g) <= steps && sps_blocks(g) < ((int64_t)1 << 31), "the sweep's schedule outgrew its table");
+  int32_t* tab = symp_table_of(pvals, G);
+  int64_t* pb = (int64_t*)(symp_sums_of(pvals, G) + steps);
+  hipLaunchKernelGGL(k_symp_sched, dim3(1), dim3(SPS_THREADS), 0, ctx->stream, g, use_flags && !g.runs ? (const unsigned char*)mfem_symp_flags_of(pvals, G) : nullptr, tab, pb,
+                     pb + steps);
+  MFEM_CHECK_LAUNCH();
+  A->symp_sW = g.W;
+  if (g_sps_record) {
+    g_sps_tab.resize((size_t)sps_table_ints(g));
+    g_sps_pb.resize((size_t)sps_blocks(g));
+    MFEM_CHECK_HIP(hipMemcpyAsync(g_sps_tab.data(), tab, sizeof(int32_t) * g_sps_tab.size(), hipMemcpyDeviceToHost, ctx->stream));
+    MFEM_CHECK_HIP(hipMemcpyAsync(g_sps_pb.data(), pb, sizeof(int64_t) * g_sps_pb.size(), hipMemcpyDeviceToHost, ctx->stream));
+    MFEM_CHECK_HIP(hipStreamSynchronize(ctx->stream));
+    g_sps_geom = g;
+  }
+  return MFEM_OK;
+}
+extern "C" int mfem_debug_symp_sched(int64_t* info, int32_t* table, int64_t cap) try {
+  MFEM_REQUIRE(info, "null argument");
+  MFEM_REQUIRE(!g_sps_tab.empty(), "no schedule was recorded (mfem_debug_set(\"symp_sched\", 2, 0) before the bind)");
+  const SpsGeom& g = g_sps_geom;
+  const int NBP = sps_nbp(g.nplanes, g.L);
+  const int64_t head[8] = {sps_blocks(g), sps_chains(g), g.R, g.W, g.L, g.NP, g.nplanes, sps_table_ints(g)};
+  for (int i = 0; i < 8; ++i) info[i] = head[i];
+  for (int c = 0; c < 8; ++c) {
+    int64_t mx = 0, sum = 0;
+    for (int jw = 0; jw < g.W; ++jw) {
+      int64_t w = 0;
+      for (int rk = 0; rk < g.R; ++rk) {
+        const int c0 = g_sps_tab[(size_t)sps_chain_at(g, c, rk, jw)], c1 = g_sps_tab[(size_t)sps_chain_at(g, c, rk, jw) + 1], pcnt = g_sps_tab[(size_t)c + 1] - g_sps_tab[(size_t)c];
+        if (c1 <= c0) continue;
+        const int seg = sps_seg_of(NBP, g.nseg, pcnt, c0), b0 = sps_seg_b0(NBP, g.nseg, seg), nbs = sps_seg_b0(NBP, g.nseg, seg + 1) - b0;
+        const int64_t a = sps_seg_off(g, seg) + (int64_t)g_sps_tab[(size_t)c] * nbs - (int64_t)pcnt * b0;
+        w += g_sps_pb[(size_t)(a + c1) - 1] - (a + c0 > 0 ? g_sps_pb[(size_t)(a + c0) - 1] : 0);
+      }
+      mx = w > mx ? w : mx;
+      sum += w;
+    }
+    info[8 + c] = mx;
+    info[16 + c] = g.W > 0 ? sum / g.W : 0;
+    info[24 + c] = g_sps_tab[(size_t)c];
+  }
+  info[32] = g_sps_tab[8];
+  info[33] = g.nseg;
+  info[34] = g.runs;
+  if (table) {
+    MFEM_REQUIRE(cap >= (int64_t)g_sps_tab.size(), "the caller's buffer is smaller than the table");
+    memcpy(table, g_sps_tab.data(), sizeof(int32_t) * g_sps_tab.size());
+  }
+  return MFEM_OK;
+} MFEM_API_CATCH("mfem_debug_symp_sched")
 
 int64_t mfem_sym_entries(const mfem_context_s* ctx, const mfem_csr_s* A, DiaKernel k) {
   if (k == DIA_SYM27) {
@@ -809,11 +1044,13 @@
     }
   }
   MFEM_CHECK_HIP(hipMemsetAsync(d_bad, 0, sizeof(int32_t), ctx->stream));
-  if (k == DIA_SYMP)
-    hipLaunchKernelGGL(symp_kernel<1>(G), dim3(symp_grid(ctx, A)), dim3(64), 0, ctx->stream, G, (const double*)pvals,
+  if (k == DIA_SYMP) {
+    const int rs = mfem_symp_schedule(ctx, A, G, pvals, false);
+    if (rs) return rs;
+    hipLaunchKernelGGL(symp_kernel<1>(G), dim3(8 * A->symp_sW), dim3(64), 0, ctx->stream, G, (const double*)pvals,
                        (const double*)nullptr, (double*)nullptr, 0.0, 0.0, (const double*)nullptr, (double*)nullptr, (const int32_t*)nullptr, d_bad,
-                       SympTail{});
-  else
+                       SympTail{}, SympSched{symp_table_of(pvals, G), nullptr, 0});
+  } else
     hipLaunchKernelGGL(k_sym27_check, dim3(ctx->num_cus * 8), dim3(MFEM_BLOCK), 0, ctx->stream, A->ell_K, (const DiaOffsets*)A->dia_dev, buf,
                        A->sym_c0 * SYM_ROWS, A->sym_c1 * SYM_ROWS, A->sym_cls, d_bad);
   MFEM_CHECK_LAUNCH();
@@ -844,19 +1081,26 @@
     SympTail tl{};
     if (a.part.part == 0 && g_ell.symp_tail) tl = SympTail{1, A->ell_K, G.rim_units > 0, A->n, A->ell_npad, lo, hi, O, A->dia_flags, A->ell_cols, A->ell_vals};
     if (a.part.part != 2) {
-      np = symp_grid(ctx, A);
+      MFEM_REQUIRE(A->symp_sW > 0, "the bound patch sweep has no schedule");
+      const int gs = 8 * A->symp_sW, ng = sps_groups(G.NR * G.NPk);
+      const SympSched sc{symp_table_of(A->symp_vals, G), symp_sums_of(A->symp_vals, G), symp_grid(ctx, A, true)};
+      np = ng + sc.vg;
       if (A->symp_CS) {
         SympConst cst{};
         memcpy(cst.v, A->symp_cst, sizeof(cst.v));
         cst.code = A->symp_ccode;
         cst.valid = 1;
-        hipLaunchKernelGGL(symp_const_kernel(G), dim3(np), dim3(64), 0, ctx->stream, G, (const double*)A->symp_vals, a.x, a.y, a.alpha, a.beta, a.dotw,
-                           a.partials, a.done_flag, tl, cst, (const uint32_t*)mfem_symp_flags_of(A->symp_vals, G));
+        hipLaunchKernelGGL(symp_const_kernel(G), dim3(gs), dim3(64), 0, ctx->stream, G, (const double*)A->symp_vals, a.x, a.y, a.alpha, a.beta, a.dotw,
+                           a.partials, a.done_flag, tl, cst, (const uint32_t*)mfem_symp_flags_of(A->symp_vals, G), sc);
       } else {
-        hipLaunchKernelGGL(symp_kernel<0>(G), dim3(np), dim3(64), 0, ctx->stream, G, (const double*)A->symp_vals, a.x, a.y, a.alpha, a.beta, a.dotw,
-                           a.partials, a.done_flag, (int32_t*)nullptr, tl);
+        hipLaunchKernelGGL(symp_kernel<0>(G), dim3(gs), dim3(64), 0, ctx->stream, G, (const double*)A->symp_vals, a.x, a.y, a.alpha, a.beta, a.dotw,
+                           a.partials, a.done_flag, (int32_t*)nullptr, tl, sc);
       }
       MFEM_CHECK_LAUNCH();
+      if (a.partials) {
+        hipLaunchKernelGGL(k_symp_fold, dim3((ng + SYMP_FOLD_WAVES - 1) / SYMP_FOLD_WAVES), dim3(64 * SYMP_FOLD_WAVES), 0, ctx->stream, G.NR * G.NPk, G.p1 - G.p0, (const double*)sc.sums, a.partials, a.done_flag);
+        MFEM_CHECK_LAUNCH();
+      }
     }
     if (a.part.part == 2 || (a.part.part == 0 && !tl.on)) {
       int go = 0;
diff --git a/metafem.jl_amd/csrc/symp_sched_decide.h b/metafem.jl_amd/csrc/symp_sched_decide.h
--- /dev/null
+++ b/metafem.jl_amd/csrc/symp_sched_decide.h
@@ -0,0 +1,122 @@
+#pragma once
+#include <stdint.h>
+
+#include "spmv_symp.h"
+
+#define SPS_PLANES 8
+#define SPS_CHAIN_BLOCKS 12
+#define SPS_PLANES_MAX 64
+#define SPS_UNFLAGGED_PS 5610000
+#define SPS_FLAGGED_PS 2000000
+#define SPS_START_UNFLAGGED_PS 2000000
+#define SPS_START_FLAGGED_PS 1000000
+#define SPS_MAX_GROUPS 1024
+#define SPS_HEAD 16
+
+struct SpsGeom {
+  int NP, nplanes, nseg;
+  int L, W;
+  int R, runs;
+  int64_t cu, cf, su, sf;
+};
+__host__ __device__ inline void sps_costs(SpsGeom& g, int ratio, int planes) {
+  g.cu = SPS_UNFLAGGED_PS;
+  g.cf = ratio >= 1000 ? ratio : ratio > 0 ? SPS_UNFLAGGED_PS / ratio : SPS_FLAGGED_PS;
+  g.su = SPS_START_UNFLAGGED_PS;
+  g.sf = SPS_START_FLAGGED_PS;
+  if (planes) {
+    g.cu = g.cf = 1;
+    g.su = g.sf = 0;
+  }
+}
+__host__ __device__ constexpr int sps_len(int L, int NP = 0, int nplanes = 0, int nseg = 1, int W = 1) {
+  if (L >= 1) return L > SPS_PLANES_MAX ? SPS_PLANES_MAX : L;
+  if (NP <= 0) return SPS_PLANES;
+  const int64_t a = (int64_t)(nplanes / nseg) * ((NP + 7) / 8) / ((int64_t)W * SPS_CHAIN_BLOCKS);
+  return a < 1 ? 1 : a > SPS_PLANES ? SPS_PLANES : (int)a;
+}
+__host__ __device__ constexpr int sps_rounds(int NP, int nseg, int W, int runs) { return runs ? (int)((((int64_t)(NP + 7) / 8) * nseg + W - 1) / W) : nseg; }
+__host__ __device__ constexpr int sps_nbp(int nplanes, int L) { return (nplanes + L - 1) / L; }
+__host__ __device__ constexpr int sps_seg_b0(int NBP, int nseg, int seg) { return (int)((int64_t)NBP * seg / nseg); }
+__host__ __device__ constexpr int64_t sps_blocks(const SpsGeom& g) { return (int64_t)g.NP * sps_nbp(g.nplanes, g.L); }
+__host__ __device__ constexpr int64_t sps_seg_off(const SpsGeom& g, int seg) { return (int64_t)g.NP * sps_seg_b0(sps_nbp(g.nplanes, g.L), g.nseg, seg); }
+__host__ __device__ constexpr int64_t sps_chains(const SpsGeom& g) { return (int64_t)8 * g.R * g.W; }
+__host__ __device__ constexpr int64_t sps_table_ints(const SpsGeom& g) { return SPS_HEAD + 2 * sps_chains(g); }
+__host__ __device__ constexpr int64_t sps_chain_at(const SpsGeom& g, int xcd, int rk, int jw) { return SPS_HEAD + 2 * (((int64_t)xcd * g.R + rk) * g.W + jw); }
+__host__ __device__ constexpr int sps_seg_of(int NBP, int nseg, int pcnt, int64_t q) {
+  int seg = 0;
+  while (seg + 1 < nseg && q >= (int64_t)pcnt * sps_seg_b0(NBP, nseg, seg + 1)) ++seg;
+  return seg;
+}
+__host__ __device__ inline void sps_block_of(const SpsGeom& g, int64_t i, int& seg, int& patch, int& blk) {
+  const int NBP = sps_nbp(g.nplanes, g.L);
+  seg = 0;
+  while (seg + 1 < g.nseg && i >= sps_seg_off(g, seg + 1)) ++seg;
+  const int b0 = sps_seg_b0(NBP, g.nseg, seg), nbs = sps_seg_b0(NBP, g.nseg, seg + 1) - b0;
+  const int64_t r = i - sps_seg_off(g, seg);
+  patch = (int)(r / nbs);
+  blk = b0 + (int)(r % nbs);
+}
+__host__ __device__ inline int64_t sps_block_cost(const SpsGeom& g, const unsigned char* flags, int patch, int blk, bool seg_first) {
+  const int pl0 = blk * g.L, pl1 = pl0 + g.L < g.nplanes ? pl0 + g.L : g.nplanes;
+  int64_t c = 0;
+  bool prev = !seg_first && flags && pl0 > 0 && flags[(int64_t)(pl0 - 1) * g.NP + patch] != 0;
+  for (int pl = pl0; pl < pl1; ++pl) {
+    const bool f = flags && flags[(int64_t)pl * g.NP + patch] != 0;
+    c += f ? g.cf : g.cu;
+    if (pl == pl0 && seg_first) c += f ? g.sf : g.su;
+    else if (!f && prev) c += g.su;
+    prev = f;
+  }
+  return c;
+}
+__host__ __device__ inline int sps_xcd_bound(const int64_t* pp, int NP, int c) {
+  if (c <= 0) return 0;
+  if (c >= 8) return NP;
+  const int64_t T = pp[NP - 1];
+  int lo = 0, hi = NP;
+  while (lo < hi) {
+    const int mid = (lo + hi) / 2;
+    if ((mid > 0 ? 8 * pp[mid - 1] : 0) >= (int64_t)c * T) hi = mid;
+    else lo = mid + 1;
+  }
+  if (lo > 0) {
+    const int64_t above = 8 * pp[lo - 1] - (int64_t)c * T, below = (int64_t)c * T - (lo > 1 ? 8 * pp[lo - 2] : 0);
+    if (below <= above) --lo;
+  }
+  return lo;
+}
+__host__ __device__ inline int sps_chain_bound(const int64_t* pb, int64_t a, int64_t b, int j, int W) {
+  const int64_t base = a > 0 ? pb[a - 1] : 0, n = b - a;
+  if (n <= 0 || j <= 0) return 0;
+  if (j >= W) return (int)n;
+  const int64_t T = pb[b - 1] - base;
+  int64_t lo = 0, hi = n;
+  while (lo < hi) {
+    const int64_t mid = (lo + hi) / 2;
+    if ((mid > 0 ? pb[a + mid - 1] - base : 0) * W >= (int64_t)j * T) hi = mid;
+    else lo = mid + 1;
+  }
+  return (int)lo;
+}
+__host__ __device__ constexpr int sps_groups(int NP) { return NP < SPS_MAX_GROUPS ? NP : SPS_MAX_GROUPS; }
+__host__ __device__ constexpr int sps_fold_lo(int NP, int gi) { return (int)((int64_t)NP * gi / sps_groups(NP)); }
+__host__ __device__ inline void sps_chain(const SpsGeom& g, const int64_t* pb, int p0, int p1, int rk, int jw, int& q0, int& q1) {
+  const int NBP = sps_nbp(g.nplanes, g.L), pcnt = p1 - p0;
+  q0 = q1 = 0;
+  if (pcnt <= 0) return;
+  if (g.runs) {
+    const int64_t k = (int64_t)rk * g.W + jw;
+    if (k >= (int64_t)pcnt * g.nseg) return;
+    const int seg = (int)(k / pcnt), b0 = sps_seg_b0(NBP, g.nseg, seg), nbs = sps_seg_b0(NBP, g.nseg, seg + 1) - b0;
+    q0 = pcnt * b0 + (int)(k % pcnt) * nbs;
+    q1 = q0 + nbs;
+    if (nbs <= 0) q0 = q1 = 0;
+    return;
+  }
+  const int seg = rk, b0 = sps_seg_b0(NBP, g.nseg, seg), nbs = sps_seg_b0(NBP, g.nseg, seg + 1) - b0;
+  const int64_t a = sps_seg_off(g, seg) + (int64_t)p0 * nbs, b = sps_seg_off(g, seg) + (int64_t)p1 * nbs;
+  q0 = pcnt * b0 + sps_chain_bound(pb, a, b, jw, g.W);
+  q1 = pcnt * b0 + sps_chain_bound(pb, a, b, jw + 1, g.W);
+  if (q1 <= q0) q0 = q1 = 0;
+}
```

New measurement: 39.10 billion DOF-updates/s (median of 6 runs). 15.0% higher.
